# POSTECH-CVLab/InstaOrder

Measured on AMD Instinct MI355X. Metric: instance-pairs/sec (fwd+bwd), higher is better.
Workload: dtype f32; 1 GPU; InstaOrderNet_o, pair-batch 256 per GPU at 256x256x5, fp32, fwd+bwd+SGD (BASELINE.json configs[1]); inputs=resident in HBM, pairs_per_gpu=256, input_size=256, parallelism=dp1, hip_graph=True, setup_steps=0, inputs_distinct=True

## Files before the change

include/instaorder_hip.h:

```cpp
#ifndef INSTAORDER_HIP_H
#define INSTAORDER_HIP_H

#include <stddef.h>
#include <stdint.h>

#ifdef __cplusplus
extern "C" {
#endif

#define IO_OK 0
#define IO_ERR_SHAPE (-1)
#define IO_ERR_WORKSPACE (-2)
#define IO_ERR_LAUNCH (-3)
#define IO_ERR_STATE (-4)
#define IO_ERR_NODEVICE (-5)

#if !defined(__HIP__) && !defined(HIP_INCLUDE_HIP_HIP_RUNTIME_API_H)
typedef void* hipStream_t;
#endif

int io_abi_version(void);
const char* io_last_error_string(void);
int io_device_count(void);
int io_set_winograd(int on);
// ... 40 lines not shown
int io_maxpool_fwd(const float* x, int N, int H, int W, int C, float* out, uint32_t* idx, hipStream_t stream);
int io_maxpool_bwd(const float* dy, const uint32_t* idx, int N, int H, int W, int C, float* dx,
                   hipStream_t stream);
int io_avgpool_fc_fwd(const float* x, int N, int HW, int C, const float* w0, const float* b0, int K0,
                      const float* w1, const float* b1, int K1, float* pooled, float* logits, hipStream_t stream);
int io_avgpool_fc_bwd(const float* dlogits, const float* pooled, int N, int HW, int C, const float* w0, int K0,
                      const float* w1, int K1, const float* relu_mask, float* dx, float* dw0, float* db0, float* dw1,
                      float* db1, hipStream_t stream);

int io_pack_planes_nhwc8(const float* const* planes, const long* sample_strides, int nplanes, int N, int H, int W,
                         float* out, hipStream_t stream);

int io_order_loss(const float* logits, int N, int B, int Kocc, int Kdep, const float* occ_target,
                  const long* depth_target, const long* is_overlap, float overlap_weight, float distinct_weight,
                  float inv_world, float* losses, float* dlogits, hipStream_t stream);

int io_sgd_momentum(float* params, const float* grads, float* momentum_buf, size_t n, float lr, float momentum,
                    float weight_decay, hipStream_t stream);

int io_adam_step(float* params, const float* grads, float* exp_avg, float* exp_avg_sq, size_t n, double lr, double beta1,
                 double beta2, float eps, float weight_decay, double bias_correction1, double bias_correction2,
                 hipStream_t stream);

typedef struct io_clip_state {
    float norm;
    float coef;
    int nonfinite;
    int reserved0;
    uint64_t steps;
    uint64_t clipped;
    uint64_t skipped;
    uint64_t reserved[3];
} io_clip_state;
int io_grad_norm_chunk_floats(void);
size_t io_grad_norm_workspace_bytes(size_t n, int nseg);
int io_grad_norm(const float* grads, size_t n, const size_t* seg_offsets, int nseg, float max_norm, void* workspace,
                 size_t workspace_bytes, double* seg_sumsq, io_clip_state* state, hipStream_t stream);
int io_sgd_momentum_clipped(float* params, const float* grads, float* momentum_buf, size_t n, float lr, float momentum,
                            float weight_decay, const io_clip_state* clip, hipStream_t stream);
int io_adam_step_clipped(float* params, const float* grads, float* exp_avg, float* exp_avg_sq, size_t n, double lr,
                         double beta1, double beta2, float eps, float weight_decay, double bias_correction1,
                         double bias_correction2, const io_clip_state* clip, hipStream_t stream);

typedef struct io_net io_net;

typedef struct io_tensor_info {
    char name[64];
    int kind;
    int ndim;
    long shape[4];
    long offset;
    long numel_storage;
    int cin_storage;
    int bn_index;
    long running_offset;
} io_tensor_info;

io_net* io_net_create(int in_channels, int n_heads, const int* head_dims);
void io_net_destroy(io_net* net);
long io_net_param_floats(const io_net* net);
long io_net_running_floats(const io_net* net);
int io_net_num_tensors(const io_net* net);
int io_net_tensor_info(const io_net* net, int i, io_tensor_info* out);
int io_net_num_logits(const io_net* net);
size_t io_net_workspace_bytes(const io_net* net, int N, int S, int training);
long io_net_activation_offset(const io_net* net, int N, int S, int which);
int io_net_forward(io_net* net, const float* params, float* running, const void* x8, int N, int S, int G,
                   int training, void* workspace, size_t workspace_bytes, float* logits, hipStream_t stream);
size_t io_net_workspace_bytes_hw(const io_net* net, int N, int H, int W);
int io_net_forward_eval_hw(io_net* net, const float* params, float* running, const void* x8, int N, int H, int W,
                           void* workspace, size_t workspace_bytes, float* logits, hipStream_t stream);

int io_net_backward_num_stages(const io_net* net);
int io_net_backward_stages(io_net* net, const float* params, float* grads, const void* x8, const float* dlogits, int N,
                           int S, int G, void* workspace, size_t workspace_bytes, int stage_lo, int stage_hi,
                           hipStream_t stream);
int io_net_backward(io_net* net, const float* params, float* grads, const void* x8, const float* dlogits, int N,
                    int S, int G, void* workspace, size_t workspace_bytes, hipStream_t stream);

#define IO_DTYPE_F32 0
#define IO_DTYPE_BF16 1
int io_net_set_dtype(io_net* net, int dtype);
int io_net_get_dtype(const io_net* net);
int io_pack_planes_nhwc8_dt(const float* const* planes, const long* sample_strides, int nplanes, int N, int H, int W,
                            void* out, int dtype, hipStream_t stream);
int io_conv2d_fwd_dt(const void* x, const void* w, void* y, int N, int H, int W, int Cin, int Cout, int R, int S,
                     int stride, int pad, int dtype_in, int dtype_out, hipStream_t stream);
int io_conv2d_dgrad_dt(const void* dy, const void* wt, void* dx, const void* add, const void* relu_mask, int N, int H,
                       int W, int Cin, int Cout, int R, int S, int stride, int pad, int dtype, hipStream_t stream);
int io_conv2d_wgrad_dt(const void* x, const void* dy, float* dw, int N, int H, int W, int Cin, int Cout, int R, int S,
                       int stride, int pad, void* workspace, size_t workspace_bytes, int dtype_in, int dtype_dy,
                       hipStream_t stream);
int io_filter_prepare(const float* w, int Cout, int taps, int Cin, void* dst, int transpose, int dtype,
                      hipStream_t stream);
int io_bn_stats_finalize_dt(const void* y, int M, int C, int G, const float* gamma, const float* beta,
                            float* running_mean, float* running_var, float momentum, float eps, float* mean,
                            float* rstd, float* scale, float* shift, float* partial, size_t partial_floats, int dtype,
                            hipStream_t stream);
int io_bn_apply_bits_dt(const void* y, int M, int C, int G, int per_group_tables, const float* mean, const float* scale,
                        const float* shift, const void* identity, const float* mean2, const float* scale2,
                        const float* shift2, void* out, uint32_t* bits, int dtype, hipStream_t stream);
int io_bn_apply_dt(const void* y, int M, int C, int G, int per_group_tables, const float* mean, const float* scale,
                   const float* shift, const void* identity, const float* mean2, const float* scale2,
                   const float* shift2, int relu, void* out, int dtype, hipStream_t stream);
int io_bn_bwd_dt(const void* dout, const void* act, const float* mask_scale, const float* mask_shift, const void* y,
                 int M, int C, int G, const float* gamma, const float* mean, const float* rstd, float* dgamma,
                 float* dbeta, void* dy, void* dz_out, float* partial, size_t partial_floats, float* coef, int dtype,
                 hipStream_t stream);

int io_gconv_pack(const float* w, int C, int cg, int taps, void* wc, void* wtc, int dtype, hipStream_t stream);
int io_gconv_unpack_grad(const float* dwc, int C, int cg, int taps, float* dw, hipStream_t stream);
int io_gconv2d_fwd(const void* x, const void* wc, void* y, int N, int H, int W, int C, int R, int S, int stride, int pad,
                   int dtype, hipStream_t stream);
int io_gconv2d_dgrad(const void* dy, const void* wtc, void* dx, int N, int H, int W, int C, int R, int S, int stride,
                     int pad, int dtype, hipStream_t stream);
size_t io_gconv2d_wgrad_workspace_bytes(int N, int H, int W, int C, int R, int S, int stride, int pad);
int io_gconv2d_wgrad(const void* x, const void* dy, float* dwc, int N, int H, int W, int C, int R, int S, int stride,
                     int pad, void* workspace, size_t workspace_bytes, int dtype, hipStream_t stream);
int io_upsample2x_bilinear_fwd(const void* x, int N, int H, int W, int C, int align_corners, void* out, int dtype,
                               hipStream_t stream);
int io_upsample2x_bilinear_bwd(const void* dy, int N, int H, int W, int C, int align_corners, void* dx, int dtype,
                               hipStream_t stream);
int io_bias_act(const void* x, const float* bias, int M, int C, int relu, void* out, int dtype, hipStream_t stream);
int io_relu_bwd(const void* dy, const void* act, size_t n, void* dx, int dtype, hipStream_t stream);
int io_add(const void* a, const void* b, size_t n, void* out, int dtype, hipStream_t stream);
size_t io_colsum_partial_floats(int M, int C);
int io_colsum(const void* x, int M, int C, float* out, float* partial, size_t partial_floats, int dtype,
              hipStream_t stream);
int io_head1_fwd(const void* x, int M, int pitch, int C, const float* w, const float* b, int relu, float* out, int dtype,
                 hipStream_t stream);
int io_head1_bwd(const float* dy, const float* out, const void* x, int M, int pitch, int C, const float* w, int relu,
                 void* dx, float* dw, float* db, float* partial, size_t partial_floats, int dtype, hipStream_t stream);
size_t io_smooth_loss_workspace_floats(int B, int H, int W);
int io_smooth_loss_fwd(const float* disp, const float* img, int B, int H, int W, float out_scale, float* loss, float* g,
                       float* workspace, size_t workspace_floats, hipStream_t stream);
int io_smooth_loss_bwd(const float* g, const float* workspace, const float* grad_out, float scale, int B, int H, int W,
                       int accumulate, float* ddisp, hipStream_t stream);
size_t io_disp_order_workspace_floats(int B, int H, int W);
int io_disp_order_count(const float* disp1, const float* disp2, const float* modal1, const float* modal2,
                        const long* depth_order1, const long* is_overlap, int B, int H, int W, int le_order,
                        float out_scale, float* out, float* workspace, size_t workspace_floats, hipStream_t stream);
size_t io_depth_errors_median_workspace_bytes(int B, int H, int W);
int io_depth_errors_median(const float* pred, const uint16_t* gt, int B, int H, int W, float gt_div, float min_depth,
                           float max_depth, double* out, float* medians, void* workspace, size_t workspace_bytes,
                           hipStream_t stream);
int io_disp_sample_points(const float* disp, int B, int H, int W, const int* points, float* values, int* decisions,
                          hipStream_t stream);
#define IO_MASK_NONZERO 0
#define IO_MASK_EQ1 1
#define IO_MASK_MAX_N 65535
int io_mask_pack(const uint8_t* masks, int n, int H, int W, int predicate, int dilate, uint32_t* bits, int64_t* stats,
                 hipStream_t stream);
int io_mask_pair_counts(const uint32_t* p_bits, int n_p, const uint32_t* q_bits, int n_q, int H, int W, int32_t* counts,
                        hipStream_t stream);
#define IO_DEPTH_SELECT_MEAN 0
#define IO_DEPTH_SELECT_MEDIAN 1
size_t io_instance_depth_select_workspace_bytes(int n, int H, int W);
int io_instance_depth_select(const float* disp, int H, int W, const uint8_t* masks, int n, int method, float* value, float* lo,
                             float* hi, int32_t* k, void* workspace, size_t workspace_bytes, hipStream_t stream);
int io_conv2d_fwd_bnstats_dt(const void* x, const void* w, void* y, int N, int H, int W, int Cin, int Cout, int R, int S,
                             int stride, int pad, int G, const float* gamma, const float* beta, float* running_mean,
                             float* running_var, float momentum, float eps, float* mean, float* rstd, float* scale,
                             float* shift, float* workspace, size_t workspace_floats, int dtype, int gw,
                             hipStream_t stream);
int io_conv2d_dgrad_bnbwd_dt(const void* dy, const void* wt, void* dz, int N, int H, int W, int Cin, int Cout, int R, int S,
                             int pad, const void* y, int G, const float* gamma, const float* mean, const float* rstd,
                             const float* scale, const float* shift, float* dgamma, float* dbeta, void* dyb,
                             float* workspace, size_t workspace_floats, int dtype, int gw, hipStream_t stream);
size_t io_stem_packed_floats(int real_channels);
size_t io_stem_wgrad_exact_workspace_bytes(int N, int H, int W, int real_channels);
int io_stem_fwd_bnstats_exact(const float* x8, const float* w, float* y, int N, int H, int W, int real_channels, int G,
                              const float* gamma, const float* beta, float* running_mean, float* running_var,
                              float momentum, float eps, float* mean, float* rstd, float* scale, float* shift,
                              float* workspace, size_t workspace_floats, float* packed, hipStream_t stream);
int io_stem_wgrad_exact(const float* x8, const float* dy, float* dw, int N, int H, int W, int real_channels,
                        void* workspace, size_t workspace_bytes, float* packed, hipStream_t stream);
int io_stem_wgrad_exact_bn(const float* x8, const float* da, const float* y, float* dw, int N, int H, int W,
                           int real_channels, int G, const float* gamma, const float* mean, const float* rstd,
                           const float* scale, const float* shift, float* dgamma, float* dbeta, float* coef,
                           float* bn_partial, size_t bn_partial_floats, void* workspace, size_t workspace_bytes,
                           float* packed, hipStream_t stream);

size_t io_bn_tile_partial_floats(int M, int C, int G);
int io_bn_bwd_coefs_dt(const void* dz, const void* y, int M, int C, int G, const float* gamma, const float* mean,
                       const float* rstd, float* dgamma, float* dbeta, float* coef, float* partial,
                       size_t partial_floats, int dtype, hipStream_t stream);
int io_bn_bwd_coefs_from_tile_partials(float* p1, float* p2, int M, int C, int G, const float* gamma, const float* mean,
                                       const float* rstd, float* dgamma, float* dbeta, float* coef, hipStream_t stream);
typedef struct io_dgrad_fused {
    const void* xb_y;
    const float* xb_coef;
    void* xb_dy_out;
    const void* add;
    const void* relu_mask;
    const void* ep_y;
    const float *ep_mean, *ep_rstd, *ep_scale, *ep_shift;
    void* ep_act_out;
    float *ep_p1, *ep_p2;
    float* wino_scratch;
    size_t wino_scratch_floats;
    const uint32_t* relu_maskbits;
} io_dgrad_fused;
int io_conv2d_dgrad_fused_dt(const void* dy, const void* wt, void* dx, int N, int H, int W, int Cin, int Cout, int R,
                             int S, int pad, int G, const io_dgrad_fused* f, int dtype, hipStream_t stream);
size_t io_conv2d_wino_scratch_floats(int Cin, int Cout);
int io_conv2d_fwd_wino(const float* x, const float* w, float* y, int N, int H, int W, int Cin, int Cout, int G,
                       const float* in_mean, const float* in_scale, const float* in_shift, const float* gamma,
                       const float* beta, float* running_mean, float* running_var, float momentum, float eps, float* mean,
                       float* rstd, float* scale, float* shift, float* workspace, size_t workspace_floats,
                       float* wino_scratch, size_t wino_floats, hipStream_t stream);
int io_conv2d_fwd_xf_dt(const void* x, const void* w, void* y, int N, int H, int W, int Cin, int Cout, int R, int S,
                        int stride, int pad, int G, const float* in_mean, const float* in_scale, const float* in_shift,
                        const float* gamma, const float* beta, float* running_mean, float* running_var, float momentum, float eps,
                        float* mean, float* rstd, float* scale, float* shift, float* workspace, size_t workspace_floats,
                        int dtype, hipStream_t stream);
int io_conv2d_fwd_resid(const float* y3, const float* identity, const float* w, float* y, float* out, int N, int H, int W,
                        int Cin, int Cout, int G, const float* in_mean, const float* in_scale, const float* in_shift,
                        const float* gamma, const float* beta, float* running_mean, float* running_var, float momentum,
                        float eps, float* mean, float* rstd, float* scale, float* shift, float* workspace,
                        size_t workspace_floats, hipStream_t stream);
int io_conv2d_fwd_resid_dt(const void* y3, const void* second, const void* w, void* y, void* out, uint32_t* out_bits, int N,
                           int H, int W, int Cin, int Cout, int G, int two, const float* ta, const float* tb, const float* tc,
                           float* tile_mean, float* tile_m2, int dtype, hipStream_t stream);
int io_set_bf16_p256_xop(int on);
int io_get_bf16_p256_xop(void);
typedef struct io_weight_desc {
    long src, dst_op, dst_t, dst_g;
    int Co, Ci, T, Cop, Cip;
} io_weight_desc;
int io_weights_prepare(const void* table, int n, const float* params, void* ops, int dtype, hipStream_t stream);
int io_weights_unpack_grads(const void* table, int n, const float* gk, float* grads, hipStream_t stream);
size_t io_stem_wgrad_bf16_workspace_bytes(void);
int io_stem_wgrad_bn_bf16(const void* x8, const void* da, const void* y, float* dw, int N, int H, int W, int G,
                          const float* gamma, const float* mean, const float* rstd, const float* scale, const float* shift,
                          float* dgamma, float* dbeta, float* coef, float* bn_partial, size_t bn_partial_floats,
                          void* workspace, size_t workspace_bytes, hipStream_t stream);
int io_debug_last_wgrad_route(void);
int io_maxpool_fwd_xf_dt(const void* x, int N, int H, int W, int C, void* out, uint32_t* idx, int G,
                         const float* in_mean, const float* in_scale, const float* in_shift, int dtype,
                         hipStream_t stream);
int io_conv2d_fwd_bias_dt(const void* x, const void* w, void* y, int N, int H, int W, int Cin, int Cout, int R, int S,
                          int stride, int pad, const float* bias, const void* add, int relu, int dtype, int gw,
                          hipStream_t stream);
int io_maxpool_fwd_dt(const void* x, int N, int H, int W, int C, void* out, uint32_t* idx, int dtype, hipStream_t stream);
int io_maxpool_bwd_dt(const void* dy, const uint32_t* idx, int N, int H, int W, int C, void* dx, int dtype,
                      hipStream_t stream);
int io_avgpool_fc_fwd_dt(const void* x, int N, int HW, int C, const float* w0, const float* b0, int K0, const float* w1,
                         const float* b1, int K1, float* pooled, float* logits, int dtype, hipStream_t stream);
int io_avgpool_fc_bwd_dt(const float* dlogits, const float* pooled, int N, int HW, int C, const float* w0, int K0,
                         const float* w1, int K1, const void* relu_mask, void* dx, float* dw0, float* db0, float* dw1,
                         float* db1, int dtype, hipStream_t stream);

typedef struct io_pair_desc {
    int64_t image_off;
    int64_t mask1_off, mask2_off;
    int32_t H, W;
    int32_t x, y, w, h;
    int32_t flip;
    int32_t interp;
} io_pair_desc;
int io_pair_planes_u8(const uint8_t* arena, size_t arena_bytes, const io_pair_desc* desc_dev,
                      const io_pair_desc* desc_host, int P, int S, const double* mean3, const double* std3, float* rgb,
                      float* modal1, float* modal2, hipStream_t stream);
int io_pair_planes_u8_hw(const uint8_t* arena, size_t arena_bytes, const io_pair_desc* desc_dev,
// ... 33 lines not shown
```

instaorder_amd/_lib.py:

```python
import ctypes as C
import os

_HERE = os.path.dirname(os.path.abspath(__file__))
LIB_PATH = os.environ.get("IO_LIB_PATH") or os.path.join(_HERE, "libinstaorder_hip.so")
_lib = None

c_float_p = C.c_void_p


def csrc_digest():
    import glob
    import hashlib
    h = hashlib.sha256()
    files = sorted(glob.glob(os.path.join(_HERE, "csrc", "*.hip")) + glob.glob(os.path.join(_HERE, "csrc", "*.h")))
    files.append(os.path.join(os.path.dirname(_HERE), "include", "instaorder_hip.h"))
    for f in files:
        h.update(os.path.basename(f).encode())
        h.update(open(f, "rb").read())
    return h.hexdigest()[:16]


class TensorInfo(C.Structure):
    _fields_ = [("name", C.c_char * 64), ("kind", C.c_int), ("ndim", C.c_int), ("shape", C.c_long * 4),
                ("offset", C.c_long), ("numel_storage", C.c_long), ("cin_storage", C.c_int),
# ... 11 lines not shown
                ("value", C.c_int32), ("out_off", C.c_int64)]


class DgradFused(C.Structure):
    _fields_ = [(n, C.c_void_p) for n in ("xb_y", "xb_coef", "xb_dy_out", "add", "relu_mask", "ep_y", "ep_mean", "ep_rstd",
                                          "ep_scale", "ep_shift", "ep_act_out", "ep_p1", "ep_p2", "wino_scratch")] + \
               [("wino_scratch_floats", C.c_size_t), ("relu_maskbits", C.c_void_p)]


class ProfEntry(C.Structure):
    _fields_ = [("name", C.c_char * 48), ("launches", C.c_long), ("total_ms", C.c_double),
                ("flops", C.c_double), ("bytes", C.c_double), ("flops_executed", C.c_double)]


class ClipState(C.Structure):
    _fields_ = [("norm", C.c_float), ("coef", C.c_float), ("nonfinite", C.c_int), ("reserved0", C.c_int),
                ("steps", C.c_uint64), ("clipped", C.c_uint64), ("skipped", C.c_uint64), ("reserved", C.c_uint64 * 3)]


_P, _I, _L, _F, _Z = C.c_void_p, C.c_int, C.c_long, C.c_float, C.c_size_t
_D = C.c_double

SIGNATURES = {
    "io_abi_version": (_I, []),
    "io_last_error_string": (C.c_char_p, []),
    "io_device_count": (_I, []),
    "io_set_winograd": (_I, [_I]),
    "io_get_winograd": (_I, []),
    "io_set_bf16_p256": (_I, [_I]),
    "io_get_bf16_p256": (_I, []),
    "io_set_bf16_p256_xop": (_I, [_I]),
    "io_get_bf16_p256_xop": (_I, []),
    "io_conv2d_fwd_resid_dt": (_I, [_P, _P, _P, _P, _P, _P, _I, _I, _I, _I, _I, _I, _I, _P, _P, _P, _P, _P, _I, _P]),
    "io_debug_last_nt_route": (_I, []),
    "io_conv2d_fwd": (_I, [_P, _P, _P, _I, _I, _I, _I, _I, _I, _I, _I, _I, _P]),
    "io_conv2d_bnstats_workspace_floats": (_Z, [_I, _I, _I, _I, _I, _I, _I, _I, _I]),
    "io_conv2d_fwd_bnstats": (_I, [_P, _P, _P, _I, _I, _I, _I, _I, _I, _I, _I, _I, _I, _P, _P, _P, _P, _F, _F, _P, _P,
                                   _P, _P, _P, _Z, _P]),
    "io_conv2d_dgrad": (_I, [_P, _P, _P, _P, _P, _I, _I, _I, _I, _I, _I, _I, _I, _I, _P]),
    "io_conv2d_dgrad_bnbwd": (_I, [_P, _P, _P, _I, _I, _I, _I, _I, _I, _I, _I, _P, _I, _P, _P, _P, _P, _P, _P, _P, _P,
                                   _P, _Z, _P]),
    "io_conv2d_wgrad_workspace_bytes": (_Z, [_I, _I, _I, _I, _I, _I, _I, _I, _I]),
    "io_conv2d_wgrad": (_I, [_P, _P, _P, _I, _I, _I, _I, _I, _I, _I, _I, _I, _P, _Z, _P]),
    "io_filter_transpose": (_I, [_P, _I, _I, _I, _P, _P]),
    "io_bn_partial_floats": (_Z, [_I, _I, _I]),
    "io_bn_stats_finalize": (_I, [_P, _I, _I, _I, _P, _P, _P, _P, _F, _F, _P, _P, _P, _P, _P, _Z, _P]),
    "io_bn_eval_prepare": (_I, [_I, _P, _P, _P, _P, _F, _P, _P, _P, _P]),
    "io_bn_apply": (_I, [_P, _I, _I, _I, _I, _P, _P, _P, _P, _P, _P, _P, _I, _P, _P]),
    "io_bn_bwd": (_I, [_P, _P, _P, _P, _P, _I, _I, _I, _P, _P, _P, _P, _P, _P, _P, _P, _Z, _P, _P]),
    "io_maxpool_fwd": (_I, [_P, _I, _I, _I, _I, _P, _P, _P]),
    "io_maxpool_bwd": (_I, [_P, _P, _I, _I, _I, _I, _P, _P]),
    "io_avgpool_fc_fwd": (_I, [_P, _I, _I, _I, _P, _P, _I, _P, _P, _I, _P, _P, _P]),
    "io_avgpool_fc_bwd": (_I, [_P, _P, _I, _I, _I, _P, _I, _P, _I, _P, _P, _P, _P, _P, _P, _P]),
    "io_pack_planes_nhwc8": (_I, [C.POINTER(C.c_void_p), C.POINTER(C.c_long), _I, _I, _I, _I, _P, _P]),
    "io_pair_planes_u8": (_I, [_P, _Z, _P, _P, _I, _I, _P, _P, _P, _P, _P, _P]),
    "io_pair_planes_u8_hw": (_I, [_P, _Z, _P, _P, _I, _I, _I, _P, _P, _P, _P, _P, _P]),
    "io_rle_decode_u8": (_I, [_P, _Z, _P, _P, _I, _P, _Z, _P]),
    "io_rle_lds_runs": (_I, []),
    "io_order_loss": (_I, [_P, _I, _I, _I, _I, _P, _P, _P, _F, _F, _F, _P, _P, _P]),
    "io_sgd_momentum": (_I, [_P, _P, _P, _Z, _F, _F, _F, _P]),
    "io_adam_step": (_I, [_P, _P, _P, _P, _Z, _D, _D, _D, _F, _F, _D, _D, _P]),
    "io_grad_norm": (_I, [_P, _Z, C.POINTER(C.c_size_t), _I, _F, _P, _Z, _P, _P, _P]),
    "io_grad_norm_workspace_bytes": (_Z, [_Z, _I]),
    "io_grad_norm_chunk_floats": (_I, []),
    "io_sgd_momentum_clipped": (_I, [_P, _P, _P, _Z, _F, _F, _F, _P, _P]),
    "io_adam_step_clipped": (_I, [_P, _P, _P, _P, _Z, _D, _D, _D, _F, _F, _D, _D, _P, _P]),
    "io_net_create": (_P, [_I, _I, C.POINTER(C.c_int)]),
    "io_net_destroy": (None, [_P]),
    "io_net_param_floats": (_L, [_P]),
    "io_net_running_floats": (_L, [_P]),
    "io_net_num_tensors": (_I, [_P]),
    "io_net_tensor_info": (_I, [_P, _I, C.POINTER(TensorInfo)]),
    "io_net_num_logits": (_I, [_P]),
    "io_net_workspace_bytes": (_Z, [_P, _I, _I, _I]),
    "io_net_workspace_bytes_hw": (_Z, [_P, _I, _I, _I]),
    "io_net_forward_eval_hw": (_I, [_P, _P, _P, _P, _I, _I, _I, _P, _Z, _P, _P]),
    "io_net_activation_offset": (_L, [_P, _I, _I, _I]),
    "io_net_forward": (_I, [_P, _P, _P, _P, _I, _I, _I, _I, _P, _Z, _P, _P]),
    "io_net_backward": (_I, [_P, _P, _P, _P, _P, _I, _I, _I, _P, _Z, _P]),
    "io_net_backward_num_stages": (_I, [_P]),
    "io_net_backward_stages": (_I, [_P, _P, _P, _P, _P, _I, _I, _I, _P, _Z, _I, _I, _P]),
    "io_net_set_dtype": (_I, [_P, _I]),
    "io_net_get_dtype": (_I, [_P]),
    "io_pack_planes_nhwc8_dt": (_I, [_P, _P, _I, _I, _I, _I, _P, _I, _P]),
    "io_conv2d_fwd_dt": (_I, [_P, _P, _P, _I, _I, _I, _I, _I, _I, _I, _I, _I, _I, _I, _P]),
    "io_conv2d_dgrad_dt": (_I, [_P, _P, _P, _P, _P, _I, _I, _I, _I, _I, _I, _I, _I, _I, _I, _P]),
    "io_conv2d_wgrad_dt": (_I, [_P, _P, _P, _I, _I, _I, _I, _I, _I, _I, _I, _I, _P, _Z, _I, _I, _P]),
    "io_filter_prepare": (_I, [_P, _I, _I, _I, _P, _I, _I, _P]),
    "io_bn_stats_finalize_dt": (_I, [_P, _I, _I, _I, _P, _P, _P, _P, _F, _F, _P, _P, _P, _P, _P, _Z, _I, _P]),
    "io_bn_apply_dt": (_I, [_P, _I, _I, _I, _I, _P, _P, _P, _P, _P, _P, _P, _I, _P, _I, _P]),
    "io_bn_apply_bits_dt": (_I, [_P, _I, _I, _I, _I, _P, _P, _P, _P, _P, _P, _P, _P, _P, _I, _P]),
    "io_bn_bwd_dt": (_I, [_P, _P, _P, _P, _P, _I, _I, _I, _P, _P, _P, _P, _P, _P, _P, _P, _Z, _P, _I, _P]),
    "io_gconv_pack": (_I, [_P, _I, _I, _I, _P, _P, _I, _P]),
    "io_gconv_unpack_grad": (_I, [_P, _I, _I, _I, _P, _P]),
    "io_gconv2d_fwd": (_I, [_P, _P, _P, _I, _I, _I, _I, _I, _I, _I, _I, _I, _P]),
    "io_gconv2d_dgrad": (_I, [_P, _P, _P, _I, _I, _I, _I, _I, _I, _I, _I, _I, _P]),
    "io_gconv2d_wgrad_workspace_bytes": (_Z, [_I, _I, _I, _I, _I, _I, _I, _I]),
    "io_gconv2d_wgrad": (_I, [_P, _P, _P, _I, _I, _I, _I, _I, _I, _I, _I, _P, _Z, _I, _P]),
    "io_upsample2x_bilinear_fwd": (_I, [_P, _I, _I, _I, _I, _I, _P, _I, _P]),
    "io_upsample2x_bilinear_bwd": (_I, [_P, _I, _I, _I, _I, _I, _P, _I, _P]),
    "io_bias_act": (_I, [_P, _P, _I, _I, _I, _P, _I, _P]),
    "io_relu_bwd": (_I, [_P, _P, _Z, _P, _I, _P]),
    "io_add": (_I, [_P, _P, _Z, _P, _I, _P]),
    "io_colsum_partial_floats": (_Z, [_I, _I]),
    "io_colsum": (_I, [_P, _I, _I, _P, _P, _Z, _I, _P]),
    "io_head1_fwd": (_I, [_P, _I, _I, _I, _P, _P, _I, _P, _I, _P]),
    "io_head1_bwd": (_I, [_P, _P, _P, _I, _I, _I, _P, _I, _P, _P, _P, _P, _Z, _I, _P]),
    "io_conv2d_fwd_bnstats_dt": (_I, [_P, _P, _P, _I, _I, _I, _I, _I, _I, _I, _I, _I, _I, _P, _P, _P, _P, _F, _F, _P,
                                      _P, _P, _P, _P, _Z, _I, _I, _P]),
    "io_conv2d_fwd_bias_dt": (_I, [_P, _P, _P, _I, _I, _I, _I, _I, _I, _I, _I, _I, _P, _P, _I, _I, _I, _P]),
    "io_stem_packed_floats": (_Z, [_I]),
    "io_stem_wgrad_exact_workspace_bytes": (_Z, [_I, _I, _I, _I]),
    "io_stem_fwd_bnstats_exact": (_I, [_P, _P, _P, _I, _I, _I, _I, _I, _P, _P, _P, _P, _F, _F, _P, _P, _P, _P, _P, _Z, _P,
                                       _P]),
    "io_stem_wgrad_exact": (_I, [_P, _P, _P, _I, _I, _I, _I, _P, _Z, _P, _P]),
    "io_stem_wgrad_exact_bn": (_I, [_P, _P, _P, _P, _I, _I, _I, _I, _I, _P, _P, _P, _P, _P, _P, _P, _P, _P, _Z, _P, _Z, _P,
                                    _P]),
    "io_stem_wgrad_bn_bf16": (_I, [_P, _P, _P, _P, _I, _I, _I, _I, _P, _P, _P, _P, _P, _P, _P, _P, _P, _Z, _P, _Z, _P]),
    "io_stem_wgrad_bf16_workspace_bytes": (_Z, []),
    "io_debug_last_wgrad_route": (_I, []),
    "io_conv2d_fwd_resid": (_I, [_P, _P, _P, _P, _P, _I, _I, _I, _I, _I, _I, _P, _P, _P, _P, _P, _P, _P, _F, _F, _P, _P, _P,
                                 _P, _P, _Z, _P]),
    "io_smooth_loss_workspace_floats": (_Z, [_I, _I, _I]),
    "io_smooth_loss_fwd": (_I, [_P, _P, _I, _I, _I, _F, _P, _P, _P, _Z, _P]),
    "io_smooth_loss_bwd": (_I, [_P, _P, _P, _F, _I, _I, _I, _I, _P, _P]),
    "io_disp_order_workspace_floats": (_Z, [_I, _I, _I]),
    "io_disp_order_count": (_I, [_P, _P, _P, _P, _P, _P, _I, _I, _I, _I, _F, _P, _P, _Z, _P]),
    "io_bn_tile_partial_floats": (_Z, [_I, _I, _I]),
    "io_bn_bwd_coefs_dt": (_I, [_P, _P, _I, _I, _I, _P, _P, _P, _P, _P, _P, _P, _Z, _I, _P]),
    "io_bn_bwd_coefs_from_tile_partials": (_I, [_P, _P, _I, _I, _I, _P, _P, _P, _P, _P, _P, _P]),
    "io_conv2d_dgrad_fused_dt": (_I, [_P, _P, _P, _I, _I, _I, _I, _I, _I, _I, _I, _I, C.POINTER(DgradFused), _I, _P]),
    "io_conv2d_dgrad_bnbwd_dt": (_I, [_P, _P, _P, _I, _I, _I, _I, _I, _I, _I, _I, _P, _I, _P, _P, _P, _P, _P, _P, _P, _P, _P,
                                      _Z, _I, _I, _P]),
    "io_prof_launches": (_I, [_P, _I]),
    "io_weights_prepare": (_I, [_P, _I, _P, _P, _I, _P]),
    "io_weights_unpack_grads": (_I, [_P, _I, _P, _P, _P]),
    "io_maxpool_fwd_xf_dt": (_I, [_P, _I, _I, _I, _I, _P, _P, _I, _P, _P, _P, _I, _P]),
    "io_conv2d_fwd_xf_dt": (_I, [_P, _P, _P, _I, _I, _I, _I, _I, _I, _I, _I, _I, _I, _P, _P, _P, _P, _P, _P, _P, _F, _F, _P,
                                 _P, _P, _P, _P, _Z, _I, _P]),
    "io_conv2d_wino_scratch_floats": (_Z, [_I, _I]),
    "io_conv2d_fwd_wino": (_I, [_P, _P, _P, _I, _I, _I, _I, _I, _I, _P, _P, _P, _P, _P, _P, _P, _F, _F, _P, _P, _P, _P, _P, _Z,
                                _P, _Z, _P]),
    "io_maxpool_fwd_dt": (_I, [_P, _I, _I, _I, _I, _P, _P, _I, _P]),
    "io_maxpool_bwd_dt": (_I, [_P, _P, _I, _I, _I, _I, _P, _I, _P]),
    "io_avgpool_fc_fwd_dt": (_I, [_P, _I, _I, _I, _P, _P, _I, _P, _P, _I, _P, _P, _I, _P]),
    "io_avgpool_fc_bwd_dt": (_I, [_P, _P, _I, _I, _I, _P, _I, _P, _I, _P, _P, _P, _P, _P, _P, _I, _P]),
    "io_depth_errors_median_workspace_bytes": (_Z, [_I, _I, _I]),
    "io_depth_errors_median": (_I, [_P, _P, _I, _I, _I, _F, _F, _F, _P, _P, _P, _Z, _P]),
    "io_disp_sample_points": (_I, [_P, _I, _I, _I, _P, _P, _P, _P]),
    "io_mask_pack": (_I, [_P, _I, _I, _I, _I, _I, _P, _P, _P]),
    "io_mask_pair_counts": (_I, [_P, _I, _P, _I, _I, _I, _P, _P]),
    "io_instance_depth_select_workspace_bytes": (_Z, [_I, _I, _I]),
    "io_instance_depth_select": (_I, [_P, _I, _I, _P, _I, _I, _P, _P, _P, _P, _P, _Z, _P]),
    "io_prof_begin": (_I, []),
    "io_prof_begin_ex": (_I, [_I]),
    "io_prof_end": (_I, [C.POINTER(ProfEntry), _I]),
}


def lib():
    global _lib
    if _lib is None:
        if not os.path.isfile(LIB_PATH):
            raise RuntimeError(
                "instaorder_amd: %s is missing -- the HIP extension has not been built "
                "(run `make -C instaorder_amd/csrc`). There is no CPU fallback." % LIB_PATH)
        _lib = C.CDLL(LIB_PATH)
        for name, (res, args) in SIGNATURES.items():
            fn = getattr(_lib, name)
            fn.restype = res
            fn.argtypes = args
    return _lib


def last_error():
    return lib().io_last_error_string().decode()


def check(rc, what):
    if rc != 0:
        raise RuntimeError("instaorder_hip %s failed (%d): %s" % (what, rc, last_error()))


_gpu_ok = None


def require_gpu():
    global _gpu_ok
    if _gpu_ok is None:
        _gpu_ok = lib().io_device_count() > 0
    if not _gpu_ok:
        raise RuntimeError("instaorder_amd: no gfx950 (MI355X) device visible; the HIP path cannot run "
                           "and there is no CPU fallback")
```

instaorder_amd/csrc/capi.hip:

```cpp
#include <stdarg.h>
#include <stdio.h>
#include <stdlib.h>
#include <string.h>

#include "io_common.h"

static thread_local char g_err[512] = "";

void io_set_error(const char* fmt, ...) {
    va_list ap;
    va_start(ap, fmt);
    vsnprintf(g_err, sizeof(g_err), fmt, ap);
    va_end(ap);
}

int io_check_launch(const char* what) {
    hipError_t e = hipGetLastError();
    if (e != hipSuccess) {
        io_set_error("%s: %s", what, hipGetErrorString(e));
        return IO_ERR_LAUNCH;
    }
    return IO_OK;
}

// ... 364 lines not shown
                                    float* db0, float* dw1, float* db1, int dtype, hipStream_t st) {
    IO_REQUIRE(dtype == IO_F32 || dtype == IO_BF16, IO_ERR_SHAPE, "avgpool_fc: unknown dtype %d", dtype);
    return io_avgpool_fc_bwd_t(dlogits, pooled, N, HW, C, w0, K0, w1, K1, relu_mask, dx, dw0, db0, dw1, db1, st, dtype);
}


extern "C" int io_conv2d_fwd_bnstats_dt(const void* x, const void* w, void* y, int N, int H, int W, int Cin, int Cout,
                                        int R, int S, int stride, int pad, int G, const float* gamma, const float* beta,
                                        float* running_mean, float* running_var, float momentum, float eps, float* mean,
                                        float* rstd, float* scale, float* shift, float* workspace,
                                        size_t workspace_floats, int dtype, int gw, hipStream_t st) {
    IO_REQUIRE(dtype == IO_F32 || dtype == IO_BF16, IO_ERR_SHAPE, "conv2d_fwd_bnstats: unknown dtype %d", dtype);
    IoConvGeom g = io_geom_fwd(N, H, W, Cin, Cout, R, S, stride, pad);
    g.gw = gw;
    const int M = N * g.Ho * g.Wo;
    IO_REQUIRE(G >= 1 && M % G == 0 && (M / G) % kIoStatTileRows == 0, IO_ERR_SHAPE,
               "conv2d_fwd_bnstats: rows per BN group (%d) must be a multiple of %d", G ? M / G : 0, kIoStatTileRows);
    const size_t need = io_conv2d_bnstats_workspace_floats(N, H, W, Cout, R, S, stride, pad, G);
    IO_REQUIRE(workspace_floats >= need, IO_ERR_WORKSPACE, "conv2d_fwd_bnstats: workspace %zu < %zu floats",
               workspace_floats, need);
    float* tmean = workspace;
    float* tm2 = workspace + need / 2;
    int rc = io_launch_conv_nt(g, x, w, y, nullptr, nullptr, Cin == 8, st, tmean, tm2, nullptr, dtype, dtype);
    if (rc) return rc;
    return io_bn_finalize_tiles(tmean, tm2, M, Cout, G, gamma, beta, running_mean, running_var, momentum, eps, mean,
                                rstd, scale, shift, st);
}


extern "C" int io_conv2d_dgrad_bnbwd_dt(const void* dy, const void* wt, void* dz, int N, int H, int W, int Cin, int Cout,
                                        int R, int S, int pad, const void* y, int G, const float* gamma, const float* mean,
                                        const float* rstd, const float* scale, const float* shift, float* dgamma,
                                        float* dbeta, void* dyb, float* workspace, size_t workspace_floats, int dtype,
                                        int gw, hipStream_t st) {
    IO_REQUIRE(dtype == IO_F32 || dtype == IO_BF16, IO_ERR_SHAPE, "conv2d_dgrad_bnbwd: unknown dtype %d", dtype);
    IO_REQUIRE(Cin % 64 == 0, IO_ERR_SHAPE, "conv2d_dgrad_bnbwd: Cin=%d must be a multiple of 64", Cin);
    const int M = N * H * W;
    IO_REQUIRE(G >= 1 && M % G == 0 && (M / G) % kIoStatTileRows == 0, IO_ERR_SHAPE,
               "conv2d_dgrad_bnbwd: rows per BN group (%d) must be a multiple of %d", G ? M / G : 0, kIoStatTileRows);
    const size_t tiles = (size_t)M / kIoStatTileRows;
    const size_t per = (tiles + tiles / 64 + G + 2) * (size_t)Cin;
    IO_REQUIRE(workspace_floats >= 2 * per + 2 * (size_t)G * Cin, IO_ERR_WORKSPACE,
               "conv2d_dgrad_bnbwd: workspace %zu < %zu floats", workspace_floats, 2 * per + 2 * (size_t)G * Cin);
    IoBwStats bw{};
    bw.y = y; bw.mean = mean; bw.rstd = rstd; bw.mscale = scale; bw.mshift = shift;
    bw.p1 = workspace; bw.p2 = workspace + per; bw.Mg = M / G;
    int rc = io_run_dgrad(dy, wt, dz, nullptr, nullptr, N, H, W, Cin, Cout, R, S, 1, pad, st, &bw, dtype, gw);
    if (rc) return rc;
    return io_bn_bwd_from_tiles(bw.p1, bw.p2, dz, y, M, Cin, G, gamma, mean, rstd, dgamma, dbeta, dyb,
                                workspace + 2 * per, st, dtype);
}

extern "C" size_t io_stem_packed_floats(int real_channels) { return (size_t)64 * io_stem_kp(49, real_channels); }
static IoConvGeom stem_geom_exact(int N, int H, int W, int cr) {
    IoConvGeom g = io_geom_fwd(N, H, W, 8, 64, 7, 7, 2, 3);
    g.cr = cr;
    return g;
}
extern "C" size_t io_stem_wgrad_exact_workspace_bytes(int N, int H, int W, int real_channels) {
    return io_conv_wgrad_partial_bytes(stem_geom_exact(N, H, W, real_channels), 1);
}
extern "C" int io_stem_fwd_bnstats_exact(const float* x8, const float* w, float* y, int N, int H, int W, int real_channels,
                                         int G, const float* gamma, const float* beta, float* running_mean,
                                         float* running_var, float momentum, float eps, float* mean, float* rstd,
                                         float* scale, float* shift, float* workspace, size_t workspace_floats,
                                         float* packed, hipStream_t st) {
    IO_REQUIRE(real_channels >= 1 && real_channels <= 8, IO_ERR_SHAPE, "stem_exact: real_channels=%d (1..8)", real_channels);
    IoConvGeom g = stem_geom_exact(N, H, W, real_channels);
    const int M = N * g.Ho * g.Wo;
    IO_REQUIRE(G >= 1 && M % G == 0 && (M / G) % kIoStatTileRows == 0, IO_ERR_SHAPE,
               "stem_exact: rows per BN group (%d) must be a multiple of %d", G ? M / G : 0, kIoStatTileRows);
    const size_t need = io_conv2d_bnstats_workspace_floats(N, H, W, 64, 7, 7, 2, 3, G);
    IO_REQUIRE(workspace_floats >= need && packed, IO_ERR_WORKSPACE, "stem_exact: workspace %zu < %zu floats",
               workspace_floats, need);
    int rc = io_stem_pack_filter(w, packed, 64, 49, real_channels, st);
    if (rc) return rc;
    float* tmean = workspace;
    float* tm2 = workspace + need / 2;
    rc = io_launch_conv_nt(g, x8, packed, y, nullptr, nullptr, 1, st, tmean, tm2);
    if (rc) return rc;
    return io_bn_finalize_tiles(tmean, tm2, M, 64, G, gamma, beta, running_mean, running_var, momentum, eps, mean, rstd,
                                scale, shift, st);
}
extern "C" int io_stem_wgrad_exact(const float* x8, const float* dy, float* dw, int N, int H, int W, int real_channels,
                                   void* ws, size_t ws_bytes, float* packed, hipStream_t st) {
    IO_REQUIRE(real_channels >= 1 && real_channels <= 8 && packed, IO_ERR_SHAPE, "stem_wgrad_exact: real_channels=%d (1..8)",
               real_channels);
    IoConvGeom g = stem_geom_exact(N, H, W, real_channels);
    int rc = io_launch_conv_wgrad(g, x8, dy, packed, (float*)ws, ws_bytes, 1, st);
    if (rc) return rc;
    return io_stem_unpack_grad(packed, dw, 64, 49, real_channels, st);
}

extern "C" int io_stem_wgrad_exact_bn(const float* x8, const float* da, const float* y, float* dw, int N, int H, int W,
                                      int real_channels, int G, const float* gamma, const float* mean, const float* rstd,
                                      const float* scale, const float* shift, float* dgamma, float* dbeta, float* coef,
                                      float* bn_partial, size_t bn_partial_floats, void* ws, size_t ws_bytes, float* packed,
                                      hipStream_t st) {
    IO_REQUIRE(real_channels >= 1 && real_channels <= 8 && packed && coef, IO_ERR_SHAPE,
               "stem_wgrad_exact_bn: real_channels=%d (1..8)", real_channels);
    IoConvGeom g = stem_geom_exact(N, H, W, real_channels);
    IO_REQUIRE(io_stem_rows_ok(g) && G >= 1 && N % G == 0, IO_ERR_SHAPE,
               "stem_wgrad_exact_bn: needs 5 real channels, 256 | H, W and G | N (else: io_bn_bwd + io_stem_wgrad_exact)");
    const int M = N * g.Ho * g.Wo;
    int rc = io_bn_bwd_coefs_t(da, y, M, 64, G, gamma, mean, rstd, dgamma, dbeta, coef, bn_partial, bn_partial_floats, st, IO_F32,
                               scale, shift);
    if (rc) return rc;
    IoStemXb xb{};
    xb.y = y;
    xb.a = coef;
    xb.b = coef + (size_t)G * 64;
    xb.c = coef + (size_t)2 * G * 64;
    xb.mean = mean;
    xb.scale = scale;
    xb.shift = shift;
    xb.G = G;
    rc = io_launch_stem_wgrad_rows(g, x8, da, packed, (float*)ws, ws_bytes, st, &xb);
    if (rc) return rc;
    return io_stem_unpack_grad(packed, dw, 64, 49, real_channels, st);
}

extern "C" size_t io_stem_wgrad_bf16_workspace_bytes(void) { return io_stem_wgrad_halo_partial_bytes(); }
extern "C" int io_stem_wgrad_bn_bf16(const void* x8, const void* da, const void* y, float* dw, int N, int H, int W, int G,
                                     const float* gamma, const float* mean, const float* rstd, const float* scale,
                                     const float* shift, float* dgamma, float* dbeta, float* coef, float* bn_partial,
                                     size_t bn_partial_floats, void* ws, size_t ws_bytes, hipStream_t st) {
    IO_REQUIRE(x8 && da && y && dw && coef && ws, IO_ERR_SHAPE, "stem_wgrad_bn_bf16: null argument");
    IoConvGeom g = io_geom_fwd(N, H, W, 8, 64, 7, 7, 2, 3);
    IO_REQUIRE(io_stem_wgrad_halo_ok(g, ws_bytes, G), IO_ERR_SHAPE,
               "stem_wgrad_bn_bf16: needs 256 x 256 inputs (128-wide output rows), G | N, io_stem_wgrad_bf16_workspace_bytes() of "
               "workspace and enough rows for the persistent blocks (else: io_bn_bwd_dt + io_conv2d_wgrad_dt)");
    const int M = N * g.Ho * g.Wo;
    int rc = io_bn_bwd_coefs_t(da, y, M, 64, G, gamma, mean, rstd, dgamma, dbeta, coef, bn_partial, bn_partial_floats, st, IO_BF16,
                               scale, shift);
    if (rc) return rc;
    IoStemXb xb{};
    xb.y = (const float*)y;
    xb.a = coef;
    xb.b = coef + (size_t)G * 64;
    xb.c = coef + (size_t)2 * G * 64;
    xb.mean = mean;
    xb.scale = scale;
    xb.shift = shift;
    xb.G = G;
    return io_launch_stem_wgrad_halo(g, x8, da, dw, (float*)ws, ws_bytes, st, &xb);
}

extern "C" size_t io_bn_tile_partial_floats(int M, int C, int G) {
    if (M <= 0 || C <= 0 || G <= 0) return 0;
    const size_t tiles = (size_t)(M + kIoStatTileRows - 1) / kIoStatTileRows;
    return (tiles + tiles / 64 + (size_t)G + 2) * (size_t)C;
}

extern "C" int io_bn_bwd_coefs_dt(const void* dz, const void* y, int M, int C, int G, const float* gamma, const float* mean,
                                  const float* rstd, float* dgamma, float* dbeta, float* coef, float* partial,
                                  size_t partial_floats, int dtype, hipStream_t st) {
    IO_REQUIRE(dtype == IO_F32 || dtype == IO_BF16, IO_ERR_SHAPE, "bn_bwd_coefs: unknown dtype %d", dtype);
    return io_bn_bwd_coefs_t(dz, y, M, C, G, gamma, mean, rstd, dgamma, dbeta, coef, partial, partial_floats, st, dtype);
}

extern "C" int io_bn_bwd_coefs_from_tile_partials(float* p1, float* p2, int M, int C, int G, const float* gamma,
                                                  const float* mean, const float* rstd, float* dgamma, float* dbeta,
                                                  float* coef, hipStream_t st) {
    return io_bn_bwd_coefs_from_tiles(p1, p2, M, C, G, gamma, mean, rstd, dgamma, dbeta, coef, st);
}

extern "C" int io_conv2d_dgrad_fused_dt(const void* dy, const void* wt, void* dx, int N, int H, int W, int Cin, int Cout,
                                        int R, int S, int pad, int G, const io_dgrad_fused* f, int dtype, hipStream_t st) {
    IO_REQUIRE(dtype == IO_F32 || dtype == IO_BF16, IO_ERR_SHAPE, "conv2d_dgrad_fused: unknown dtype %d", dtype);
    IO_REQUIRE(f != nullptr, IO_ERR_SHAPE, "conv2d_dgrad_fused: the option struct is required");
    IO_REQUIRE(Cin % 64 == 0, IO_ERR_SHAPE, "conv2d_dgrad_fused: Cin=%d must be a multiple of 64", Cin);
    const int M = N * H * W;
    const bool grouped = f->xb_coef || f->ep_y;
    IO_REQUIRE(!grouped || (G >= 1 && M % G == 0 && (M / G) % kIoStatTileRows == 0), IO_ERR_SHAPE,
               "conv2d_dgrad_fused: rows per BN group (%d) must be a multiple of %d", G ? M / G : 0, kIoStatTileRows);
    IO_REQUIRE(!f->xb_coef || f->xb_y, IO_ERR_SHAPE, "conv2d_dgrad_fused: xb_coef needs xb_y");
    IO_REQUIRE(!f->ep_y || (f->ep_mean && f->ep_rstd && f->ep_p1 && f->ep_p2 && (f->ep_scale == nullptr) == (f->ep_shift == nullptr)),
               IO_ERR_SHAPE, "conv2d_dgrad_fused: ep_y needs ep_mean / ep_rstd / ep_p1 / ep_p2 (and scale / shift as a pair)");
    IO_REQUIRE(!f->ep_act_out || (f->ep_y && f->ep_scale), IO_ERR_SHAPE,
               "conv2d_dgrad_fused: ep_act_out needs ep_y with ep_scale / ep_shift");
    IoBwStats bw{};
    if (f->ep_y) {
        bw.y = f->ep_y; bw.mean = f->ep_mean; bw.rstd = f->ep_rstd; bw.mscale = f->ep_scale; bw.mshift = f->ep_shift;
        bw.p1 = f->ep_p1; bw.p2 = f->ep_p2; bw.Mg = M / G; bw.a_out = f->ep_act_out;
    }
    if (f->xb_coef) {
        const size_t gs = (size_t)G * Cout;
        bw.xb_y = f->xb_y; bw.xb_a = f->xb_coef; bw.xb_b = f->xb_coef + gs; bw.xb_c = f->xb_coef + 2 * gs;
        bw.xb_out = f->xb_dy_out; bw.xb_Mg = M / G;
    }
    if (f->wino_scratch) {
        IO_REQUIRE(f->wino_scratch_floats >= io_conv2d_wino_scratch_floats(Cin, Cout), IO_ERR_WORKSPACE,
                   "conv2d_dgrad_fused: wino_scratch %zu < %zu floats", f->wino_scratch_floats,
                   io_conv2d_wino_scratch_floats(Cin, Cout));
        bw.wino_u = f->wino_scratch;
    }
    if (f->relu_maskbits) {
        IO_REQUIRE(f->relu_mask && Cin % 32 == 0, IO_ERR_SHAPE,
                   "conv2d_dgrad_fused: relu_maskbits goes WITH relu_mask (the same mask, one bit per element), 32 | Cin");
        bw.maskbits = f->relu_maskbits;
    }
    return io_run_dgrad(dy, wt, dx, f->add, f->relu_mask, N, H, W, Cin, Cout, R, S, 1, pad, st,
// ... 120 lines not shown
```

instaorder_amd/csrc/io_common.h:

```cpp
#pragma once
#include <hip/hip_runtime.h>
#include <stdint.h>
#include <stddef.h>

#include "../../include/instaorder_hip.h"

void io_set_error(const char* fmt, ...);
int io_check_launch(const char* what);

#define IO_REQUIRE(cond, code, ...)        \
    do {                                   \
        if (!(cond)) {                     \
            io_set_error(__VA_ARGS__);     \
            return (code);                 \
        }                                  \
    } while (0)

static inline int io_cdiv(long a, long b) { return (int)((a + b - 1) / b); }

#include <atomic>
static inline int io_device_cu_count() {
    static std::atomic<int> cache[64];
    int dev = 0;
    if (hipGetDevice(&dev) != hipSuccess || dev < 0 || dev >= 64) return 256;
// ... 89 lines not shown
    const void* y;
    const float *mean, *rstd, *mscale, *mshift;
    float *p1, *p2;
    int Mg;
    void* a_out;
    const float* bias;
    int relu;
    const float *in_mean, *in_scale, *in_shift;
    int in_Mg;
    const void* xb_y;
    const float *xb_a, *xb_b, *xb_c;
    void* xb_out;
    int xb_Mg;
    int xb_res;
    uint32_t* xb_bits;
    float* wino_u;
    const uint32_t* maskbits;
};

bool io_wino_on();

int io_launch_conv_nt(const IoConvGeom& g, const void* in, const void* wgt, void* out, const void* add,
                      const void* mask, int stem, hipStream_t st, float* st_mean = nullptr,
                      float* st_m2 = nullptr, const IoBwStats* bw = nullptr, int dt_in = IO_F32,
                      int dt_out = IO_F32);
bool io_conv_p256_takes_xop(long M, int Ci, int Co, int Mg);
int io_launch_conv_p256(const IoConvGeom& g, const void* in, const void* wgt, void* out, const void* add, const void* mask,
                        hipStream_t st, float* st_mean, float* st_m2, const IoBwStats* bw, size_t in_bytes,
                        unsigned w_bytes, size_t out_bytes);
int io_bf16_persist_mode();
int io_launch_conv_halo3(const IoConvGeom& g, const void* in, const void* wgt, void* out, const void* add, const void* mask,
                         hipStream_t st, float* st_mean, float* st_m2, const IoBwStats* bw, size_t in_bytes,
                         unsigned w_bytes, size_t out_bytes);
int io_launch_conv_stem_halo(const IoConvGeom& g, const void* in, const void* wgt, void* out, hipStream_t st, float* st_mean,
                             float* st_m2, const IoBwStats* bw, size_t in_bytes, unsigned w_bytes, size_t out_bytes);
int io_bn_bwd_from_tiles(float* p1, float* p2, const void* dz, const void* y, int M, int C, int G,
                         const float* gamma, const float* mean, const float* rstd, float* dgamma, float* dbeta,
                         void* dy, float* coef, hipStream_t st, int dt = IO_F32);
int io_bn_bwd_coefs_from_tiles(float* p1, float* p2, int M, int C, int G, const float* gamma, const float* mean,
                               const float* rstd, float* dgamma, float* dbeta, float* coef, hipStream_t st);
int io_bn_bwd_coefs_t(const void* dz, const void* y, int M, int C, int G, const float* gamma, const float* mean,
                      const float* rstd, float* dgamma, float* dbeta, float* coef, float* partial,
                      size_t partial_floats, hipStream_t st, int dt, const float* mask_scale = nullptr,
                      const float* mask_shift = nullptr);
int io_bn_stats_finalize_t(const void* y, int M, int C, int G, const float* gamma, const float* beta,
                           float* running_mean, float* running_var, float momentum, float eps, float* mean,
                           float* rstd, float* scale, float* shift, float* partial, size_t partial_floats,
                           hipStream_t st, int dt);
int io_bn_apply_t(const void* y, int M, int C, int G, int per_group_tables, const float* mean, const float* scale,
                  const float* shift, const void* identity, const float* mean2, const float* scale2,
                  const float* shift2, int relu, void* out, hipStream_t st, int dt, uint32_t* bits = nullptr);
int io_bn_bwd_t(const void* dout, const void* act, const float* mask_scale, const float* mask_shift, const void* y,
                int M, int C, int G, const float* gamma, const float* mean, const float* rstd, float* dgamma,
                float* dbeta, void* dy, void* dz_out, float* partial, size_t partial_floats, float* coef,
                hipStream_t st, int dt);
int io_maxpool_fwd_t(const void* x, int N, int H, int W, int C, void* out, uint32_t* idx, hipStream_t st, int dt,
                     const float* xs = nullptr, const float* xh = nullptr, int G = 1, const float* xm = nullptr);
int io_maxpool_bwd_t(const void* dy, const uint32_t* idx, int N, int H, int W, int C, void* dx, hipStream_t st, int dt);
int io_avgpool_fc_fwd_t(const void* x, int N, int HW, int C, const float* w0, const float* b0, int K0,
                        const float* w1, const float* b1, int K1, float* pooled, float* logits, hipStream_t st,
                        int dt);
int io_avgpool_fc_bwd_t(const float* dlogits, const float* pooled, int N, int HW, int C, const float* w0, int K0,
                        const float* w1, int K1, const void* relu_mask, void* dx, float* dw0, float* db0, float* dw1,
                        float* db1, hipStream_t st, int dt);
int io_pack_planes_t(const float* const* planes, const long* sample_strides, int nplanes, int N, int H, int W,
                     void* out, hipStream_t st, int dt);
int io_filter_prepare_t(const float* w, int O, int T, int C, void* dst, int transpose, hipStream_t st, int dt);
int io_stem_pack_filter(const float* w, float* wp, int O, int T, int cr, hipStream_t st);
int io_stem_unpack_grad(const float* dwp, float* dw, int O, int T, int cr, hipStream_t st);
int io_bn_resid2_tables(const float* mean3, const float* scale3, const float* shift3, const float* meand,
                        const float* scaled, const float* shiftd, int G, int C, float* coef, hipStream_t st);
constexpr int kIoStatTileRows = 128;
int io_bn_finalize_tiles(float* tile_mean, float* tile_m2, int M, int C, int G, const float* gamma,
                         const float* beta, float* running_mean, float* running_var, float momentum, float eps,
                         float* mean, float* rstd, float* scale, float* shift, hipStream_t st);
int io_launch_conv_wgrad(const IoConvGeom& g, const void* in, const void* dy, float* dw, float* partial,
                         size_t partial_bytes, int stem, hipStream_t st, int dt_in = IO_F32, int dt_dy = IO_F32);
size_t io_conv_wgrad_partial_bytes(const IoConvGeom& g, int stem);

IoConvGeom io_geom_fwd(int N, int H, int W, int Cin, int Cout, int R, int S, int stride, int pad);
bool io_stem_rows_ok(const IoConvGeom& g);
int io_launch_stem_rows(const IoConvGeom& g, const float* x8, const float* wp, float* out, float* st_mean, float* st_m2,
                        const float* bias, int relu, hipStream_t st);
int io_stem_wgrad_rows_max_blocks();
struct IoStemXb {
    const float *y, *a, *b, *c, *mean, *scale, *shift;
    int G, tiles_per_group;
};
int io_launch_stem_wgrad_rows(const IoConvGeom& g, const float* x8, const float* dy, float* dwp, float* partial,
                              size_t partial_bytes, hipStream_t st, const IoStemXb* xb = nullptr);
size_t io_stem_wgrad_halo_partial_bytes();
bool io_stem_wgrad_halo_ok(const IoConvGeom& g, size_t partial_bytes, int G);
int io_launch_stem_wgrad_halo(const IoConvGeom& g, const void* x8, const void* dz, float* dw, float* partial, size_t partial_bytes,
                              hipStream_t st, const IoStemXb* xb);
size_t io_wgrad_halo3_partial_bytes();
bool io_wgrad_halo3_shape(const IoConvGeom& g);
int io_launch_conv_wgrad_halo3(const IoConvGeom& g, const void* x, const void* dy, float* dw, float* partial, size_t partial_bytes,
                               hipStream_t st);
int io_splitk_reduce(const float* partial, float* dst, size_t n4, int splits, hipStream_t st);
struct IoFilterTable {
    static constexpr int kMax = 64;
    int n;
    int start[kMax + 1];
    int O[kMax], T[kMax], C[kMax];
    unsigned off[kMax];
};
int io_filter_table_add(IoFilterTable& tab, long off, int O, int T, int C);
int io_filter_transpose_all(const IoFilterTable& tab, const float* params, void* wt_all, hipStream_t st, int dt);
IoConvGeom io_geom_dgrad(int N, int H, int W, int Cin, int Cout, int R, int S, int stride, int pad, int ph, int pw);
int io_run_dgrad(const void* dy, const void* wt, void* dx, const void* add, const void* mask, int N, int H,
                 int W, int Cin, int Cout, int R, int S, int stride, int pad, hipStream_t st,
                 const IoBwStats* bw = nullptr, int dt = IO_F32, int gw = 0);

enum IoProfClass {
    IO_PROF_CONV_NT128 = 0, IO_PROF_CONV_NT64, IO_PROF_CONV_STEM, IO_PROF_WGRAD, IO_PROF_WGRAD_STEM,
    IO_PROF_BN_STATS, IO_PROF_BN_APPLY, IO_PROF_BN_BWD, IO_PROF_POOL_HEAD, IO_PROF_TRANSPOSE, IO_PROF_PACK,
    IO_PROF_LOSS, IO_PROF_SGD, IO_PROF_CONV_WINO, IO_PROF_WGRAD_WINO, IO_PROF_ADAM, IO_PROF_GRAD_NORM,
    IO_PROF_RLE, IO_PROF_NCLASS
};
struct IoProfScope {
    int idx;
    hipStream_t st;
    IoProfScope(int cls, double flops, double bytes, hipStream_t stream, double flops_exec = -1.0);
    ~IoProfScope();
};
```

instaorder_amd/csrc/misc.hip:

```cpp
#include "io_common.h"

#ifndef IO_POOL_ROWS
#define IO_POOL_ROWS 1
#endif

namespace {

constexpr int kThreads = 256;

template <typename T> __device__ __forceinline__ f32x4 ld4(const T* p) { return io_ldv(p); }
template <typename T> __device__ __forceinline__ void st4(T* p, f32x4 v) { io_stv(p, v); }
__device__ __forceinline__ float ld1(const float* p) { return *p; }
__device__ __forceinline__ float ld1(const bf16_t* p) { return io_bf2f(*p); }
__device__ __forceinline__ void st1(float* p, float v) { *p = v; }
__device__ __forceinline__ void st1(bf16_t* p, float v) { *p = io_f2bf(v); }

int ew_blocks(size_t n) {
    size_t b = (n + kThreads - 1) / kThreads;
    return (int)(b > 8192 ? 8192 : (b ? b : 1));
}

struct PackArgs {
    const float* plane[5];
    long stride[5];
// ... 871 lines not shown
extern "C" size_t io_grad_norm_workspace_bytes(size_t n, int nseg) {
    return ((n + kNormChunk - 1) / kNormChunk + (size_t)(nseg > 0 ? nseg : 0)) * sizeof(double);
}

extern "C" int io_grad_norm(const float* grads, size_t n, const size_t* seg_offsets, int nseg, float max_norm,
                            void* workspace, size_t workspace_bytes, double* seg_sumsq, io_clip_state* state,
                            hipStream_t st) {
    static_assert(sizeof(io_clip_state) == 64, "io_clip_state is a 64-byte record");
    NormTable tab;
    const int rc = norm_table(tab, n, seg_offsets, nseg);
    if (rc != IO_OK) return rc;
    IO_REQUIRE(max_norm > 0.f, IO_ERR_SHAPE, "grad_norm: max_norm=%g must be > 0 (+inf: measure only)", (double)max_norm);
    IO_REQUIRE(seg_sumsq && state && (grads || n == 0), IO_ERR_SHAPE, "grad_norm: null pointer");
    const size_t blocks = (size_t)tab.start[nseg];
    IO_REQUIRE(blocks == 0 || (workspace && workspace_bytes >= blocks * sizeof(double)), IO_ERR_SHAPE,
               "grad_norm: workspace of %zu bytes, %zu needed", workspace_bytes, blocks * sizeof(double));
    IO_REQUIRE(((uintptr_t)grads & 15) == 0 && ((uintptr_t)workspace & 7) == 0, IO_ERR_SHAPE,
               "grad_norm: grads must be 16-byte aligned, the workspace 8-byte aligned");
    IoProfScope prof(IO_PROF_GRAD_NORM, 3.0 * n, 4.0 * n, st);
    if (blocks)
        hipLaunchKernelGGL(grad_norm_partial_kernel, dim3((unsigned)blocks), dim3(kThreads), 0, st, tab, grads,
                           (double*)workspace);
    hipLaunchKernelGGL(grad_norm_fold_kernel, dim3(1), dim3(kThreads), 0, st, tab, (const double*)workspace, seg_sumsq,
                       max_norm, state);
    return io_check_launch("grad_norm");
}

int io_filter_prepare_t(const float* w, int O, int T, int C, void* dst, int transpose, hipStream_t st, int dt) {
    IoProfScope prof(IO_PROF_TRANSPOSE, 0.0, (4.0 + io_dtype_bytes(dt)) * O * T * C, st);
    if (transpose) {
        dim3 grid(io_cdiv(C, 32), io_cdiv(O, 32), T);
        if (dt == IO_BF16)
            hipLaunchKernelGGL(filter_transpose_kernel<bf16_t>, grid, dim3(256), 0, st, w, O, T, C, (bf16_t*)dst);
        else
            hipLaunchKernelGGL(filter_transpose_kernel<float>, grid, dim3(256), 0, st, w, O, T, C, (float*)dst);
    } else {
        IO_REQUIRE(dt == IO_BF16 && ((size_t)O * T * C) % 4 == 0, IO_ERR_SHAPE, "filter_prepare: nothing to do");
        const size_t n4 = (size_t)O * T * C / 4;
        hipLaunchKernelGGL(cast_bf16_kernel, dim3(ew_blocks(n4)), dim3(kThreads), 0, st, w, (bf16_t*)dst, n4);
    }
    return io_check_launch("filter_prepare");
}

int io_filter_table_add(IoFilterTable& tab, long off, int O, int T, int C) {
    IO_REQUIRE(tab.n < IoFilterTable::kMax && off >= 0 && off < (1L << 32) && off % 8 == 0 && O > 0 && T > 0 && C > 0,
               IO_ERR_SHAPE, "filter table: entry %d (offset %ld, %d x %d x %d)", tab.n, off, O, T, C);
    const int l = tab.n++;
    tab.off[l] = (unsigned)off;
    tab.O[l] = O; tab.T[l] = T; tab.C[l] = C;
    tab.start[l + 1] = tab.start[l] + io_cdiv(C, 32) * io_cdiv(O, 32) * T;
    return IO_OK;
}

int io_filter_transpose_all(const IoFilterTable& tab, const float* params, void* wt_all, hipStream_t st, int dt) {
    if (tab.n == 0) return IO_OK;
    double elems = 0.0;
    for (int l = 0; l < tab.n; ++l) elems += (double)tab.O[l] * tab.T[l] * tab.C[l];
    IoProfScope prof(IO_PROF_TRANSPOSE, 0.0, (4.0 + io_dtype_bytes(dt)) * elems, st);
    const dim3 grid((unsigned)tab.start[tab.n]);
    if (dt == IO_BF16)
        hipLaunchKernelGGL(filter_transpose_all_kernel<bf16_t>, grid, dim3(256), 0, st, tab, params, (bf16_t*)wt_all);
    else
        hipLaunchKernelGGL(filter_transpose_all_kernel<float>, grid, dim3(256), 0, st, tab, params, (float*)wt_all);
    return io_check_launch("filter_transpose_all");
}

namespace {
__global__ __launch_bounds__(256) void stem_pack_filter_kernel(const float* __restrict__ w, float* __restrict__ wp,
                                                              int O, int T, int cr, int kp) {
    const int idx = blockIdx.x * 256 + threadIdx.x;
    if (idx >= O * kp) return;
    const int o = idx / kp, k = idx - o * kp;
    const int tp = k / cr, ch = k - tp * cr;
    wp[idx] = tp < T ? w[((size_t)o * T + tp) * 8 + ch] : 0.f;
}
__global__ __launch_bounds__(256) void stem_unpack_grad_kernel(const float* __restrict__ dwp, float* __restrict__ dw,
                                                              int O, int T, int cr, int kp) {
    const int idx = blockIdx.x * 256 + threadIdx.x;
    if (idx >= O * T * 8) return;
    const int ch = idx & 7, ot = idx >> 3;
    const int o = ot / T, tp = ot - o * T;
    dw[idx] = ch < cr ? dwp[(size_t)o * kp + tp * cr + ch] : 0.f;
}
}

int io_stem_pack_filter(const float* w, float* wp, int O, int T, int cr, hipStream_t st) {
    const int kp = io_stem_kp(T, cr);
    hipLaunchKernelGGL(stem_pack_filter_kernel, dim3(io_cdiv((long)O * kp, 256)), dim3(256), 0, st, w, wp, O, T, cr, kp);
    return io_check_launch("stem_pack_filter");
}

int io_stem_unpack_grad(const float* dwp, float* dw, int O, int T, int cr, hipStream_t st) {
    const int kp = io_stem_kp(T, cr);
    hipLaunchKernelGGL(stem_unpack_grad_kernel, dim3(io_cdiv((long)O * T * 8, 256)), dim3(256), 0, st, dwp, dw, O, T,
                       cr, kp);
    return io_check_launch("stem_unpack_grad");
}

extern "C" int io_filter_transpose(const float* w, int O, int T, int C, float* wt, hipStream_t st) {
    return io_filter_prepare_t(w, O, T, C, wt, 1, st, IO_F32);
}
```

instaorder_amd/csrc/net.hip:

```cpp
#include <stdio.h>
#include <string.h>

#include <vector>

#include "io_common.h"

namespace {

constexpr int kMaxGroups = 8;
constexpr float kBnEps = 1e-5f, kBnMomentum = 0.1f;

struct ConvL {
    int cin, cout, k, stride, pad, cin_store;
    long w_off;
};
struct BnL {
    int C;
    long g_off, b_off, run_off;
    int index;
};
struct Block {
    ConvL c1, c2, c3, cd;
    BnL b1, b2, b3, bd;
    bool down;
    int stride, inC, planes;
};

inline size_t align_up(size_t v, size_t a) { return (v + a - 1) / a * a; }

}

struct io_net {
    int dtype = IO_F32;
    int in_ch, n_heads, head_dims[2];
    ConvL stem;
    BnL bn1;
    std::vector<Block> blocks;
    long fcw_off[2], fcb_off[2];
    long param_floats, running_floats;
    int n_bn;
    long bn_channels;
    std::vector<io_tensor_info> tensors;
};

namespace {

void add_tensor(io_net* net, const char* name, int kind, int ndim, const long* shape, long numel_storage,
                int cin_storage, long* off_out, int bn_index = -1, long run_off = -1) {
    io_tensor_info t;
    memset(&t, 0, sizeof(t));
    snprintf(t.name, sizeof(t.name), "%s", name);
    t.kind = kind;
    t.ndim = ndim;
    for (int i = 0; i < ndim; ++i) t.shape[i] = shape[i];
    t.offset = net->param_floats;
    t.numel_storage = numel_storage;
    t.cin_storage = cin_storage;
    t.bn_index = bn_index;
    t.running_offset = run_off;
    *off_out = net->param_floats;
    net->param_floats = (long)align_up((size_t)(net->param_floats + numel_storage), 64);
    net->tensors.push_back(t);
}

ConvL add_conv(io_net* net, const char* name, int cout, int cin, int k, int stride, int pad) {
    ConvL c;
    c.cin = cin; c.cout = cout; c.k = k; c.stride = stride; c.pad = pad;
    c.cin_store = (cin % 32 == 0) ? cin : 8;
    char nm[64];
    snprintf(nm, sizeof(nm), "%s.weight", name);
    const long shape[4] = {cout, cin, k, k};
    add_tensor(net, nm, 0, 4, shape, (long)cout * k * k * c.cin_store, c.cin_store, &c.w_off);
    return c;
}

BnL add_bn(io_net* net, const char* name, int C) {
    BnL b;
    b.C = C;
    b.index = net->n_bn++;
    b.run_off = net->running_floats;
    net->running_floats += 2L * C;
    net->bn_channels += C;
    char nm[64];
    const long shape[1] = {C};
    snprintf(nm, sizeof(nm), "%s.weight", name);
    add_tensor(net, nm, 1, 1, shape, C, C, &b.g_off, b.index, b.run_off);
    snprintf(nm, sizeof(nm), "%s.bias", name);
    add_tensor(net, nm, 2, 1, shape, C, C, &b.b_off, b.index, b.run_off);
    return b;
}

constexpr size_t kNoBuf = ~(size_t)0;
struct BlockBufs {
    size_t y1, a1, y2, a2, y3, yd, out;
    size_t bits;
};
struct Plan {
    size_t y0, a0, p0, idx0, pooled;
    std::vector<BlockBufs> blk;
    size_t tables;
    size_t bn_partial, bn_partial_floats, coef;
    size_t tile_mean, tile_m2;
    size_t gbuf[5];
    size_t aside;
    size_t wt, wg_partial, wg_partial_bytes;
    size_t wop;
    size_t stem_wp, stem_dwp;
    size_t wt_all;
    size_t wfold, fbias;
    size_t wino_u;
    size_t total;
};

struct Arena {
    size_t top = 0;
    size_t take(size_t bytes) {
// ... 98 lines not shown
        p.wg_partial_bytes = 0;
    }
    p.total = a.top;
    return p;
}

struct FoldDesc {
    long w_off, g_off, b_off, run_off, bias_off;
    int rows, rowlen;
};
struct FoldTable {
    int n;
    FoldDesc d[56];
};
template <typename T>
__global__ __launch_bounds__(256) void fold_bn_kernel(FoldTable t, const float* __restrict__ params,
                                                     const float* __restrict__ running, float eps,
                                                     T* __restrict__ wout, float* __restrict__ bias) {
    const FoldDesc d = t.d[blockIdx.y];
    for (int row = blockIdx.x; row < d.rows; row += gridDim.x) {
        const float s = params[d.g_off + row] / sqrtf(running[d.run_off + d.rows + row] + eps);
        if (threadIdx.x == 0) bias[d.bias_off + row] = params[d.b_off + row] - running[d.run_off + row] * s;
        const float* src = params + d.w_off + (size_t)row * d.rowlen;
        T* dst = wout + d.w_off + (size_t)row * d.rowlen;
        for (int k = threadIdx.x; k < d.rowlen; k += 256) {
            if constexpr (sizeof(T) == 2) dst[k] = io_f2bf(src[k] * s);
            else dst[k] = src[k] * s;
        }
    }
}

#define IO_TRY(expr)            \
    do {                        \
        int rc_ = (expr);       \
        if (rc_) return rc_;    \
    } while (0)

struct Tables {
    float *mean, *rstd, *scale, *shift;
};

struct Ctx {
    const io_net* net;
    const float* params;
    float* running;
    float* grads;
    char* ws;
    Plan plan;
    int N, S, G;
    int SW;
    bool training;
    hipStream_t st;
    std::vector<long> chan_prefix;

    float* buf(size_t off) const { return reinterpret_cast<float*>(ws + off); }
    void* act(size_t off) const { return ws + off; }
    int dt() const { return net->dtype; }
    const void* wop(long w_off) const {
        return net->dtype == IO_BF16 ? (const void*)(reinterpret_cast<const bf16_t*>(ws + plan.wop) + w_off)
                                     : (const void*)(params + w_off);
    }
    const void* wfold(long w_off) const {
        return net->dtype == IO_BF16 ? (const void*)(reinterpret_cast<const bf16_t*>(ws + plan.wfold) + w_off)
                                     : (const void*)(reinterpret_cast<const float*>(ws + plan.wfold) + w_off);
    }
    float* fbias(const BnL& b) const { return buf(plan.fbias) + chan_prefix[b.index]; }
    Tables tables(const BnL& b) const {
        float* base = buf(plan.tables) + (size_t)4 * kMaxGroups * chan_prefix[b.index];
        const size_t gs = (size_t)kMaxGroups * b.C;
        return Tables{base, base + gs, base + 2 * gs, base + 3 * gs};
    }
};

bool stem_exact(const Ctx& c, const ConvL& L) { return L.cin_store == 8 && c.net->dtype == IO_F32; }

int conv_fwd(const Ctx& c, const ConvL& L, const void* x, void* y, int H, bool stats = false, const BnL* xf = nullptr,
             int Mout = 0, const BnL* xr = nullptr, const void* xr_id = nullptr, void* xr_out = nullptr,
             bool xr_two = false, uint32_t* xr_bits = nullptr) {
    IoConvGeom g = io_geom_fwd(c.N, H, H, L.cin_store, L.cout, L.k, L.k, L.stride, L.pad);
    const bool stem = L.cin_store == 8;
    const void* w = c.wop(L.w_off);
    if (stem_exact(c, L)) {
        g.cr = L.cin;
        IO_TRY(io_stem_pack_filter(c.params + L.w_off, c.buf(c.plan.stem_wp), L.cout, L.k * L.k, L.cin, c.st));
        w = c.buf(c.plan.stem_wp);
    }
    IoBwStats ep{};
    if (xf) {
        Tables t = c.tables(*xf);
        ep.in_mean = t.mean;
        ep.in_scale = t.scale;
        ep.in_shift = t.shift;
        ep.in_Mg = Mout / c.G;
    }
    const bool wino = c.plan.wino_u != kNoBuf && L.k == 3 && L.stride == 1 && c.dt() == IO_F32;
    if (wino) ep.wino_u = c.buf(c.plan.wino_u);
    if (xr) {
        Tables t = c.tables(*xr);
        ep.xb_y = xr_id;
        ep.xb_a = t.scale;
        ep.xb_b = t.mean;
        ep.xb_c = t.shift;
        ep.xb_out = xr_out;
        ep.xb_Mg = Mout / c.G;
        ep.xb_res = 1;
        ep.xb_bits = xr_bits;
        if (xr_two) {
            const size_t gs = (size_t)c.G * xr->C;
            ep.xb_a = c.buf(c.plan.coef);
            ep.xb_b = c.buf(c.plan.coef) + gs;
            ep.xb_c = c.buf(c.plan.coef) + 2 * gs;
            ep.xb_res = 2;
        }
    }
    return io_launch_conv_nt(g, x, w, y, nullptr, nullptr, stem, c.st,
                             stats ? c.buf(c.plan.tile_mean) : nullptr, stats ? c.buf(c.plan.tile_m2) : nullptr,
                             (xf || xr || wino) ? &ep : nullptr, c.dt(), c.dt());
}

int bn_prepare(const Ctx& c, const BnL& b, const void* y, int M, bool from_tiles = false) {
    Tables t = c.tables(b);
    if (c.training && from_tiles)
        return io_bn_finalize_tiles(c.buf(c.plan.tile_mean), c.buf(c.plan.tile_m2), M, b.C, c.G,
                                    c.params + b.g_off, c.params + b.b_off, c.running + b.run_off,
                                    c.running + b.run_off + b.C, kBnMomentum, kBnEps, t.mean, t.rstd, t.scale,
                                    t.shift, c.st);
    if (c.training)
        return io_bn_stats_finalize_t(y, M, b.C, c.G, c.params + b.g_off, c.params + b.b_off, c.running + b.run_off,
                                      c.running + b.run_off + b.C, kBnMomentum, kBnEps, t.mean, t.rstd, t.scale,
                                      t.shift, c.buf(c.plan.bn_partial), c.plan.bn_partial_floats, c.st, c.dt());
    return io_bn_eval_prepare(b.C, c.params + b.g_off, c.params + b.b_off, c.running + b.run_off,
                              c.running + b.run_off + b.C, kBnEps, t.mean, t.scale, t.shift, c.st);
}

int conv_bn(const Ctx& c, const ConvL& L, const BnL& b, const void* x, void* y, int Hin, int Mout,
            const BnL* xf = nullptr, const BnL* xr = nullptr, const void* xr_id = nullptr, void* xr_out = nullptr,
            bool xr_two = false, uint32_t* xr_bits = nullptr) {
    const bool fuse = c.training && (Mout / c.G) % kIoStatTileRows == 0;
    IO_TRY(conv_fwd(c, L, x, y, Hin, fuse, xf, Mout, xr, xr_id, xr_out, xr_two, xr_bits));
    return bn_prepare(c, b, y, Mout, fuse);
}

#ifndef IO_XB_BF16_MAXP
#define IO_XB_BF16_MAXP 64
#endif
#ifndef IO_XB_BF16_L1
#define IO_XB_BF16_L1 1
#endif
int out_rows(const Ctx& c, size_t i) {
    int H = c.S / 4;
    for (size_t k = 0; k <= i; ++k) H /= c.net->blocks[k].stride;
    return c.N * H * H;
}
int xr_route(const Ctx& c, size_t i) {
    if (!c.training || i + 1 >= c.net->blocks.size()) return 0;
    const Block& b = c.net->blocks[i];
    const int Mout = out_rows(c, i);
    if (Mout % c.G != 0 || (Mout / c.G) % kIoStatTileRows != 0) return 0;
    if (c.net->dtype == IO_F32) return 1;
    if (IO_XB_BF16_L1 && b.planes <= IO_XB_BF16_MAXP) return 1;
    return io_conv_p256_takes_xop(Mout, b.planes * 4, c.net->blocks[i + 1].planes, Mout / c.G) ? 2 : 0;
}

uint32_t* bits_of(const Ctx& c, size_t i) {
    const size_t off = c.plan.blk[i].bits;
    return (c.training && off != kNoBuf) ? reinterpret_cast<uint32_t*>(c.ws + off) : nullptr;
// ... 326 lines not shown
        if (stage_of[ii] < stage_lo || stage_of[ii] >= stage_hi) {
            have_tiles = ii > 0 && tiles_ok(c, Min);
            void* t = Gd; Gd = Ge; Ge = t;
            continue;
        }
        const void* xin = ii == 0 ? c.act(p.p0) : c.act(p.blk[ii - 1].out);
        const void* xmask = ii == 0 ? nullptr : xin;
        const bool x3p = c.net->dtype == IO_BF16 && b.planes > IO_XB_BF16_MAXP && tiles_ok(c, Mout) &&
                         io_conv_p256_takes_xop(Mout, b.planes * 4, b.planes, Mout / c.G);
        const bool x3 = xb_ok(c, Mout) || x3p ||
                        (IO_XB_BF16_L1 && c.net->dtype == IO_BF16 && b.planes <= IO_XB_BF16_MAXP && tiles_ok(c, Mout));
        const bool f3 = fuse_in(c, Mout), f2 = f3 && b.stride == 1;
        const bool x1d = b.stride == 1 && xb_ok(c, Min) && tiles_ok(c, Mout);
        const bool x1s = b.stride != 1 && xb_ok(c, Min) && bb.a1 != kNoBuf;
        const bool x1 = x1d || x1s;
        if (x3)
            IO_TRY(bn_back_coefs(c, b.b3, Gd, c.act(bb.y3), Mout, have_tiles));
        else if (have_tiles)
            IO_TRY(bn_back_tiles(c, b.b3, Gd, c.act(bb.y3), Mout, Ga));
        else
            IO_TRY(bn_back(c, b.b3, Gd, 0, nullptr, c.act(bb.y3), Mout, Ga, nullptr));
        have_tiles = false;
        void* As = f3 ? c.act(p.aside) : nullptr;
        if (!f3 && !x3) IO_TRY(conv_wgrad(c, b.c3, c.act(bb.a2), Ga, Ho));
        IO_TRY(dgrad_then_bn(c, b.c3, x3 ? Gd : Ga, Gb, Ho, b.b2, c.act(bb.y2), Mout, Gc, f3 ? As : nullptr,
                             x3 ? &b.b3 : nullptr, c.act(bb.y3), Mout, Ga));
        if (f3 || x3) IO_TRY(conv_wgrad(c, b.c3, f3 ? As : c.act(bb.a2), Ga, Ho));
        if (!f2) IO_TRY(conv_wgrad(c, b.c2, c.act(bb.a1), Gc, H));
        if (x1s)
            IO_TRY(conv_dgrad(c, b.c2, Gc, Ga, nullptr, c.act(bb.a1), H));
        else
            IO_TRY(dgrad_then_bn(c, b.c2, Gc, Ga, H, b.b1, c.act(bb.y1), Min, x1 ? nullptr : Gb, f2 ? As : nullptr));
        if (f2) IO_TRY(conv_wgrad(c, b.c2, As, Gc, H));
        if (!x1) IO_TRY(conv_wgrad(c, b.c1, xin, Gb, H));
        const void* partial = Gd;
        if (b.down && x3 && !x3p) {
            IO_TRY(bn_back_coefs(c, b.bd, Gd, c.act(bb.yd), Mout, false));
            IoBwStats bw{};
            xb_fill(c, bw, b.bd, c.act(bb.yd), Mout, Gc);
            IO_TRY(conv_dgrad(c, b.cd, Gd, Ge, nullptr, nullptr, H, &bw));
            IO_TRY(conv_wgrad(c, b.cd, xin, Gc, H));
            partial = Ge;
        } else if (b.down) {
            IO_TRY(bn_back(c, b.bd, Gd, 0, nullptr, c.act(bb.yd), Mout, Gc, nullptr));
            IO_TRY(conv_wgrad(c, b.cd, xin, Gc, H));
            IO_TRY(conv_dgrad(c, b.cd, Gc, Ge, nullptr, nullptr, H));
            partial = Ge;
        }
        if (x1) IO_TRY(bn_back_coefs(c, b.b1, Ga, c.act(bb.y1), Min, x1d));
        {
            IoBwStats bw{};
            const bool carry = ii > 0 && tiles_ok(c, Min);
            if (carry) bw = bw_for(c, net->blocks[ii - 1].b3, c.act(p.blk[ii - 1].y3), Min, false);
            if (x1) xb_fill(c, bw, b.b1, c.act(bb.y1), Min, Gb);
            const uint32_t* mbits = (ii > 0 && xmask && bits_written(c, ii - 1)) ? bits_of(c, ii - 1) : nullptr;
            if (mbits) bw.maskbits = mbits;
            IO_TRY(conv_dgrad(c, b.c1, x1 ? Ga : Gb, Ge, partial, xmask, H, (carry || x1 || mbits) ? &bw : nullptr));
            have_tiles = carry;
        }
        if (x1) IO_TRY(conv_wgrad(c, b.c1, xin, Gb, H));
        void* t = Gd; Gd = Ge; Ge = t;
    }
    if (stage_hi < kBwdStages) return IO_OK;
    IO_TRY(io_maxpool_bwd_t(Gd, reinterpret_cast<const uint32_t*>(c.ws + p.idx0), c.N, H0, H0, 64, Ge, c.st, c.dt()));
    {
        IoConvGeom g = io_geom_fwd(c.N, c.S, c.S, 8, 64, 7, 7, 2, 3);
        g.cr = net->stem.cin;
        if (stem_exact(c, net->stem) && io_stem_rows_ok(g) && c.N % c.G == 0) {
            const BnL& b = net->bn1;
            Tables t = c.tables(b);
            IO_TRY(io_bn_bwd_coefs_t(Ge, c.act(p.y0), c.N * H0 * H0, b.C, c.G, c.params + b.g_off, t.mean, t.rstd,
                                     c.grads + b.g_off, c.grads + b.b_off, c.buf(c.plan.coef), c.buf(c.plan.bn_partial),
                                     c.plan.bn_partial_floats, c.st, c.dt(), t.scale, t.shift));
            const size_t gs = (size_t)c.G * b.C;
            IoStemXb xb{};
            xb.y = (const float*)c.act(p.y0);
            xb.a = c.buf(c.plan.coef);
            xb.b = c.buf(c.plan.coef) + gs;
            xb.c = c.buf(c.plan.coef) + 2 * gs;
            xb.mean = t.mean;
            xb.scale = t.scale;
            xb.shift = t.shift;
            xb.G = c.G;
            IO_TRY(io_launch_stem_wgrad_rows(g, (const float*)x8, (const float*)Ge, c.buf(c.plan.stem_dwp),
                                             c.buf(c.plan.wg_partial), c.plan.wg_partial_bytes, c.st, &xb));
            return io_stem_unpack_grad(c.buf(c.plan.stem_dwp), c.grads + net->stem.w_off, net->stem.cout, 49,
                                       net->stem.cin, c.st);
        }
    }
    if (c.net->dtype == IO_BF16) {
        IoConvGeom g = io_geom_fwd(c.N, c.S, c.S, 8, 64, 7, 7, 2, 3);
        if (io_stem_wgrad_halo_ok(g, c.plan.wg_partial_bytes, c.G)) {
            const BnL& b = net->bn1;
            Tables t = c.tables(b);
            IO_TRY(io_bn_bwd_coefs_t(Ge, c.act(p.y0), c.N * H0 * H0, b.C, c.G, c.params + b.g_off, t.mean, t.rstd,
                                     c.grads + b.g_off, c.grads + b.b_off, c.buf(c.plan.coef), c.buf(c.plan.bn_partial),
                                     c.plan.bn_partial_floats, c.st, c.dt(), t.scale, t.shift));
            const size_t gs = (size_t)c.G * b.C;
            IoStemXb xb{};
            xb.y = (const float*)c.act(p.y0);
            xb.a = c.buf(c.plan.coef);
            xb.b = c.buf(c.plan.coef) + gs;
            xb.c = c.buf(c.plan.coef) + 2 * gs;
            xb.mean = t.mean;
            xb.scale = t.scale;
            xb.shift = t.shift;
            xb.G = c.G;
            return io_launch_stem_wgrad_halo(g, x8, Ge, c.grads + net->stem.w_off, c.buf(c.plan.wg_partial),
                                             c.plan.wg_partial_bytes, c.st, &xb);
        }
    }
    IO_TRY(bn_back(c, net->bn1, Ge, 1, nullptr, c.act(p.y0), c.N * H0 * H0, Ga, nullptr));
    IO_TRY(conv_wgrad(c, net->stem, x8, Ga, c.S));
    return IO_OK;
}

}

extern "C" io_net* io_net_create(int in_channels, int n_heads, const int* head_dims) {
    if (in_channels < 1 || in_channels > 5 || n_heads < 1 || n_heads > 2) {
        io_set_error("io_net_create: in_channels=%d (1..5), n_heads=%d (1..2)", in_channels, n_heads);
        return nullptr;
    }
    for (int i = 0; i < n_heads; ++i)
        if (head_dims[i] < 1 || head_dims[i] > 4 || (n_heads == 2 && i == 0 && head_dims[i] != 2)) {
            io_set_error("io_net_create: unsupported head dims");
            return nullptr;
        }
    io_net* net = new io_net();
    net->in_ch = in_channels;
    net->n_heads = n_heads;
    net->head_dims[0] = head_dims[0];
    net->head_dims[1] = n_heads > 1 ? head_dims[1] : 0;
    net->param_floats = 0;
    net->running_floats = 0;
    net->n_bn = 0;
    net->bn_channels = 0;
    net->stem = add_conv(net, "conv1", 64, in_channels, 7, 2, 3);
    net->stem.cin_store = 8;
    net->bn1 = add_bn(net, "bn1", 64);
    const int layers[4] = {3, 4, 6, 3}, planes[4] = {64, 128, 256, 512};
    int inC = 64;
    for (int li = 0; li < 4; ++li)
        for (int bi = 0; bi < layers[li]; ++bi) {
            Block b;
            char nm[64];
            b.planes = planes[li];
            b.inC = inC;
            b.stride = (bi == 0 && li > 0) ? 2 : 1;
            b.down = bi == 0;
            snprintf(nm, sizeof(nm), "layer%d.%d.conv1", li + 1, bi);
            b.c1 = add_conv(net, nm, b.planes, inC, 1, 1, 0);
            snprintf(nm, sizeof(nm), "layer%d.%d.bn1", li + 1, bi);
            b.b1 = add_bn(net, nm, b.planes);
            snprintf(nm, sizeof(nm), "layer%d.%d.conv2", li + 1, bi);
            b.c2 = add_conv(net, nm, b.planes, b.planes, 3, b.stride, 1);
            snprintf(nm, sizeof(nm), "layer%d.%d.bn2", li + 1, bi);
            b.b2 = add_bn(net, nm, b.planes);
            snprintf(nm, sizeof(nm), "layer%d.%d.conv3", li + 1, bi);
            b.c3 = add_conv(net, nm, b.planes * 4, b.planes, 1, 1, 0);
            snprintf(nm, sizeof(nm), "layer%d.%d.bn3", li + 1, bi);
            b.b3 = add_bn(net, nm, b.planes * 4);
            if (b.down) {
                snprintf(nm, sizeof(nm), "layer%d.%d.downsample.0", li + 1, bi);
                b.cd = add_conv(net, nm, b.planes * 4, inC, 1, b.stride, 0);
                snprintf(nm, sizeof(nm), "layer%d.%d.downsample.1", li + 1, bi);
                b.bd = add_bn(net, nm, b.planes * 4);
            }
            inC = b.planes * 4;
            net->blocks.push_back(b);
        }
    const char* hn1[1] = {"fc"};
    const char* hn2[2] = {"fc_occ", "fc_depth"};
    for (int i = 0; i < n_heads; ++i) {
        char nm[64];
        const char* base = n_heads == 1 ? hn1[0] : hn2[i];
        const long ws[2] = {head_dims[i], 2048};
        snprintf(nm, sizeof(nm), "%s.weight", base);
        add_tensor(net, nm, 3, 2, ws, (long)head_dims[i] * 2048, 2048, &net->fcw_off[i]);
        const long bs[1] = {head_dims[i]};
        snprintf(nm, sizeof(nm), "%s.bias", base);
        add_tensor(net, nm, 4, 1, bs, head_dims[i], head_dims[i], &net->fcb_off[i]);
    }
    return net;
}

extern "C" void io_net_destroy(io_net* net) { delete net; }
extern "C" int io_net_set_dtype(io_net* net, int dtype) {
    IO_REQUIRE(dtype == IO_F32 || dtype == IO_BF16, IO_ERR_SHAPE, "io_net_set_dtype: unknown dtype %d", dtype);
    net->dtype = dtype;
    return IO_OK;
}
extern "C" int io_net_get_dtype(const io_net* net) { return net->dtype; }
extern "C" long io_net_param_floats(const io_net* net) { return net->param_floats; }
extern "C" long io_net_running_floats(const io_net* net) { return net->running_floats; }
extern "C" int io_net_num_tensors(const io_net* net) { return (int)net->tensors.size(); }
extern "C" int io_net_num_logits(const io_net* net) { return net->head_dims[0] + net->head_dims[1]; }

extern "C" int io_net_tensor_info(const io_net* net, int i, io_tensor_info* out) {
    IO_REQUIRE(i >= 0 && i < (int)net->tensors.size(), IO_ERR_SHAPE, "tensor index %d out of range", i);
    *out = net->tensors[i];
    return IO_OK;
}

static int check_shape(int N, int S, int G) {
    IO_REQUIRE(S >= 32 && S % 32 == 0, IO_ERR_SHAPE, "input size S=%d must be a multiple of 32", S);
    IO_REQUIRE(N >= 1 && G >= 1 && G <= kMaxGroups && N % G == 0, IO_ERR_SHAPE, "N=%d G=%d (G<=%d, G | N)", N, G,
               kMaxGroups);
    IO_REQUIRE((double)N * S * S < 2.0e9, IO_ERR_SHAPE, "N=%d x S=%d: more than 2^31 input pixels", N, S);
    return IO_OK;
}

extern "C" size_t io_net_workspace_bytes(const io_net* net, int N, int S, int training) {
    if (check_shape(N, S, 1)) return 0;
    return make_plan(net, N, S, training != 0).total;
}

extern "C" long io_net_activation_offset(const io_net* net, int N, int S, int which) {
    if (check_shape(N, S, 1)) return -1;
    const Plan p = make_plan(net, N, S, true);
    const int nb = (int)net->blocks.size();
    if (which == 0) return (long)p.y0;
    if (which == 1) {
        io_set_error("io_net_activation_offset: relu(bn1(.)) is not stored (it is evaluated inside the pooling kernel)");
        return -1;
    }
    if (which == 2) return (long)p.p0;
    if (which >= 3 && which < 3 + nb) return (long)p.blk[which - 3].out;
    io_set_error("io_net_activation_offset: which=%d (0..%d)", which, 2 + nb);
    return -1;
}

static void fill_ctx(Ctx& c, io_net* net, const float* params, float* running, float* grads, int N, int S, int G,
                     bool training, void* ws, hipStream_t st, int SW = 0) {
    c.net = net;
    c.params = params;
    c.running = running;
    c.grads = grads;
    c.ws = (char*)ws;
    c.N = N; c.S = S; c.G = G;
    c.SW = SW > 0 ? SW : S;
    c.training = training;
    c.st = st;
    c.plan = make_plan(net, N, S, training, c.SW);
    c.chan_prefix.assign(net->n_bn, 0);
    std::vector<int> Cs(net->n_bn, 0);
    Cs[net->bn1.index] = net->bn1.C;
    for (const Block& b : net->blocks) {
        Cs[b.b1.index] = b.b1.C;
        Cs[b.b2.index] = b.b2.C;
        Cs[b.b3.index] = b.b3.C;
        if (b.down) Cs[b.bd.index] = b.bd.C;
    }
    long acc = 0;
    for (int i = 0; i < net->n_bn; ++i) { c.chan_prefix[i] = acc; acc += Cs[i]; }
}

extern "C" int io_net_forward(io_net* net, const float* params, float* running, const void* x8, int N, int S,
                              int G, int training, void* ws, size_t ws_bytes, float* logits, hipStream_t st) {
    IO_TRY(check_shape(N, S, G));
    IO_REQUIRE(training || G == 1, IO_ERR_SHAPE, "eval forward uses running statistics: G must be 1");
    Ctx c;
    fill_ctx(c, net, params, running, nullptr, N, S, G, training != 0, ws, st);
    IO_REQUIRE(ws_bytes >= c.plan.total, IO_ERR_WORKSPACE, "io_net_forward: workspace %zu < %zu bytes", ws_bytes,
               c.plan.total);
    return run_forward(c, x8, logits);
}

static int check_shape_hw(int N, int H, int W) {
    IO_REQUIRE(H >= 32 && H % 32 == 0 && W >= 32 && W % 32 == 0, IO_ERR_SHAPE,
               "input %d x %d: both sides must be multiples of 32 (five stride-2 stages)", H, W);
    IO_REQUIRE(N >= 1 && (double)N * H * W < 2.0e9, IO_ERR_SHAPE, "N=%d x %d x %d: more than 2^31 input pixels", N, H, W);
    return IO_OK;
}
extern "C" size_t io_net_workspace_bytes_hw(const io_net* net, int N, int H, int W) {
    if (check_shape_hw(N, H, W)) return 0;
// ... 38 lines not shown
```

instaorder_amd/csrc/stem.hip:

```cpp
#include <hip/hip_runtime.h>

#include <type_traits>

#include "io_common.h"

#ifndef IO_STEM_ABLATE
#define IO_STEM_ABLATE 0
#endif

typedef float f32x2 __attribute__((ext_vector_type(2)));
typedef float f32x4 __attribute__((ext_vector_type(4)));
typedef float f32x16 __attribute__((ext_vector_type(16)));

namespace {
constexpr int kCR = 5;
constexpr int kPW = 262;
constexpr int kPitch = kPW * kCR;
constexpr int kKB = 36;
constexpr int kBImg = 7 * 64 * kKB;
constexpr int kPix = 7 * kPW;
constexpr int kNT = 512;
constexpr int kRounds = (kPix + kNT - 1) / kNT;
constexpr int kPatch = kRounds * kNT * kCR;
constexpr int kRed = 2 * 4 * 64 * 2;
// ... 71 lines not shown
    const float bv = bias ? bias[ch] : 0.f;
    const float floor_v = relu ? 0.f : -__builtin_inff();
    f32x16 acc, pacc;
#pragma unroll
    for (int r = 0; r < 16; ++r) pacc[r] = 0.f;
    int cur = 0;
    auto mma_row = [&](int r) {
        const float* ar = sP + cur * kPatch + a_lane + r * kPitch;
        const float* br = b_lane + r * 64 * kKB;
#pragma unroll
        for (int q = 0; q < 4; ++q) {
            const f32x2 a0 = *reinterpret_cast<const f32x2*>(ar + 8 * q + 4 * h);
            const f32x2 a1 = *reinterpret_cast<const f32x2*>(ar + 8 * q + 4 * h + 2);
            const f32x4 b = *reinterpret_cast<const f32x4*>(br + 8 * q + 4 * h);
            acc = __builtin_amdgcn_mfma_f32_32x32x2f32(a0.x, b.x, acc, 0, 0, 0);
            acc = __builtin_amdgcn_mfma_f32_32x32x2f32(a0.y, b.y, acc, 0, 0, 0);
            acc = __builtin_amdgcn_mfma_f32_32x32x2f32(a1.x, b.z, acc, 0, 0, 0);
            acc = __builtin_amdgcn_mfma_f32_32x32x2f32(a1.y, b.w, acc, 0, 0, 0);
        }
        const f32x2 a = *reinterpret_cast<const f32x2*>(ar + 32 + 2 * h);
        const f32x2 b = *reinterpret_cast<const f32x2*>(br + 32 + 2 * h);
        acc = __builtin_amdgcn_mfma_f32_32x32x2f32(a.x, b.x, acc, 0, 0, 0);
        acc = __builtin_amdgcn_mfma_f32_32x32x2f32(a.y, b.y, acc, 0, 0, 0);
    };
    auto park = [&](int t) {
        float s = 0.f;
#pragma unroll
        for (int r = 0; r < 16; ++r) s += pacc[r];
        s += __shfl_xor(s, 32, 64);
        const float m = s * (1.f / 32.f);
        float q = 0.f;
#pragma unroll
        for (int r = 0; r < 16; ++r) q += (pacc[r] - m) * (pacc[r] - m);
        q += __shfl_xor(q, 32, 64);
        *reinterpret_cast<f32x2*>(sR + (((t & 1) * 4 + rg) * 64 + ch) * 2) = f32x2{m, q};
    };
    auto merge = [&](int t) {
        const float* rr = sR + ((t & 1) * 4 * 64 + ch) * 2;
        const f32x2 p0 = *reinterpret_cast<const f32x2*>(rr), p1 = *reinterpret_cast<const f32x2*>(rr + 128);
        const f32x2 p2 = *reinterpret_cast<const f32x2*>(rr + 256), p3 = *reinterpret_cast<const f32x2*>(rr + 384);
        const float mean = ((p0.x + p1.x) + (p2.x + p3.x)) * 0.25f;
        const float d0 = p0.x - mean, d1 = p1.x - mean, d2 = p2.x - mean, d3 = p3.x - mean;
        st_mean[(size_t)t * 64 + ch] = mean;
        st_m2[(size_t)t * 64 + ch] = ((p0.y + p1.y) + (p2.y + p3.y)) + 32.f * ((d0 * d0 + d1 * d1) + (d2 * d2 + d3 * d3));
    };
    auto store_half = [&](int t, int half) {
        float* o = out + ((size_t)t * 128 + rg * 32 + 4 * h) * 64 + ch;
#pragma unroll
        for (int r = 8 * half; r < 8 * half + 8; ++r) {
            const float v = pacc[r] + bv;
            o[(size_t)((r & 3) + 8 * (r >> 2)) * 64] = v < floor_v ? floor_v : v;
        }
    };
    auto body = [&](auto steady, int t) {
        constexpr bool STEADY = decltype(steady)::value;
        const bool have = STEADY || t < t_hi, prev = STEADY || (t > t_lo && t <= t_hi), prev2 = STEADY || t > t_lo + 1;
        const bool more = STEADY || t + 1 < t_hi;
        if (more && !(IO_STEM_ABLATE & 2)) fetch();
        __builtin_amdgcn_sched_barrier(0);
#pragma unroll
        for (int r = 0; r < 16; ++r) acc[r] = 0.f;
        if (have) mma_row(0);
        if (STATS && prev && !(IO_STEM_ABLATE & 4)) park(t - 1);
        if (have) mma_row(1);
        if (STATS && prev2 && !(IO_STEM_ABLATE & 4)) merge(t - 2);
        if (have) mma_row(2);
        if (prev && (!(IO_STEM_ABLATE & 1) || pacc[0] == 123.456f)) store_half(t - 1, 0);
        if (have) mma_row(3);
        if (prev && (!(IO_STEM_ABLATE & 1) || pacc[0] == 123.456f)) store_half(t - 1, 1);
        if (have) mma_row(4);
        if (more && !(IO_STEM_ABLATE & 2)) stage(cur ^ 1);
        if (have) mma_row(5);
        if (have) mma_row(6);
        __syncthreads();
        pacc = acc;
        cur ^= 1;
    };
    for (int t = t_lo; t <= t_hi + 1; ++t) {
        if (t > t_lo + 1 && t + 1 < t_hi) body(std::true_type{}, t);
        else body(std::false_type{}, t);
    }
}

constexpr int kWPitch = 1315;
constexpr int kWPatch = kRounds * kNT * kCR + 40;
constexpr int kWDy = 128 * 64;
constexpr size_t kWLds = (size_t)2 * (kWPatch + kWDy) * sizeof(float);

template <bool XB>
__global__ __launch_bounds__(kNT, 1) void stem_wgrad_rows_kernel(const float* __restrict__ x8, const float* __restrict__ dy,
                                                                 float* __restrict__ partial, int Hi, int Wi, int Ho, int Wo,
                                                                 int ntiles, int per_block, IoStemXb xb) {
    extern __shared__ __attribute__((aligned(16))) float smem[];
    float* sP = smem;
    float* sD = smem + 2 * kWPatch;
    const int tid = threadIdx.x, lane = tid & 63, wave = tid >> 6;
    const int l32 = lane & 31, h = lane >> 5;
    const int t_lo = blockIdx.x * per_block, t_hi = min(ntiles, t_lo + per_block);
    const int cbn = Wo >> 7;

    float pr[kRounds][kCR];
    f32x4 dr[4], yr[4], tb[6];
    int p_r[kRounds], p_c[kRounds], p_off[kRounds], p_dst[kRounds];
    bool p_ok[kRounds];
#pragma unroll
    for (int i = 0; i < kRounds; ++i) {
        const int p = tid + i * kNT;
        p_r[i] = p / kPW;
        p_c[i] = p - p_r[i] * kPW;
        p_off[i] = (p_r[i] * Wi + p_c[i]) * 8;
        p_dst[i] = p_r[i] * kWPitch + p_c[i] * kCR;
        if (p >= kPix || p_c[i] >= kPW - 1) p_r[i] = 1 << 20;
    }
    int f_cb = t_lo % cbn, f_ho = (t_lo / cbn) % Ho, f_n = (t_lo / cbn) / Ho;
    const float* f_dy = dy + (size_t)t_lo * kWDy + tid * 4;
    const float* f_y = XB ? xb.y + (size_t)t_lo * kWDy + tid * 4 : nullptr;
    int f_t = t_lo;
    auto fetch = [&]() {
        const int hi0 = 2 * f_ho - 3, wi0 = 256 * f_cb - 3;
        const float* base = x8 + (((ptrdiff_t)f_n * Hi + hi0) * Wi + wi0) * 8;
        if (++f_cb == cbn) {
            f_cb = 0;
            if (++f_ho == Ho) {
                f_ho = 0;
                ++f_n;
            }
        }
#pragma unroll
        for (int i = 0; i < kRounds; ++i) {
            const bool ok = (unsigned)(hi0 + p_r[i]) < (unsigned)Hi && (unsigned)(wi0 + p_c[i]) < (unsigned)Wi;
            const float* src = ok ? base + p_off[i] : x8;
            const f32x4 v = *reinterpret_cast<const f32x4*>(src);
            pr[i][0] = v.x; pr[i][1] = v.y; pr[i][2] = v.z; pr[i][3] = v.w;
            pr[i][4] = src[4];
            p_ok[i] = ok;
        }
#pragma unroll
        for (int i = 0; i < 4; ++i) dr[i] = *reinterpret_cast<const f32x4*>(f_dy + i * kNT * 4);
        f_dy += kWDy;
        if constexpr (XB) {
#pragma unroll
            for (int i = 0; i < 4; ++i) yr[i] = *reinterpret_cast<const f32x4*>(f_y + i * kNT * 4);
            f_y += kWDy;
            const int go = (f_t / xb.tiles_per_group) * 64 + (tid & 15) * 4;
            ++f_t;
            tb[0] = *reinterpret_cast<const f32x4*>(xb.a + go);
            tb[1] = *reinterpret_cast<const f32x4*>(xb.b + go);
            tb[2] = *reinterpret_cast<const f32x4*>(xb.c + go);
            tb[3] = *reinterpret_cast<const f32x4*>(xb.mean + go);
            tb[4] = *reinterpret_cast<const f32x4*>(xb.scale + go);
            tb[5] = *reinterpret_cast<const f32x4*>(xb.shift + go);
        }
    };
    auto stage = [&](int buf) {
        float* dst = sP + buf * kWPatch;
#pragma unroll
        for (int i = 0; i < kRounds; ++i)
#pragma unroll
            for (int c = 0; c < kCR; ++c) dst[p_dst[i] + c] = p_ok[i] ? pr[i][c] : 0.f;
        float* dd = sD + buf * kWDy + tid * 4;
#pragma unroll
        for (int i = 0; i < 4; ++i) {
            f32x4 v = dr[i];
            if constexpr (XB) {
#pragma unroll
                for (int e = 0; e < 4; ++e) {
                    const float act = __builtin_fmaf(yr[i][e] - tb[3][e], tb[4][e], tb[5][e]);
                    const float dz = act > 0.f ? v[e] : 0.f;
                    v[e] = __builtin_fmaf(tb[0][e], dz, __builtin_fmaf(tb[1][e], yr[i][e], tb[2][e]));
                }
            }
            *reinterpret_cast<f32x4*>(dd + i * kNT * 4) = v;
        }
    };

    fetch();
    stage(0);
    __syncthreads();

    const int j = wave * 32 + l32;
    const int jr = min(j, 7 * 7 * kCR - 1) / (7 * kCR), jk = min(j, 7 * 7 * kCR - 1) - jr * 7 * kCR;
    const int b_lane = jr * kWPitch + jk + 2 * kCR * h;
    const int a_lane = h * 64 + l32;
    f32x16 acc0, acc1;
#pragma unroll
    for (int r = 0; r < 16; ++r) acc0[r] = acc1[r] = 0.f;
    int cur = 0;
    auto mma_tile = [&]() {
        const float* pb = sP + cur * kWPatch + b_lane;
        const float* pa = sD + cur * kWDy + a_lane;
        float fb[2][8], fa0[2][8], fa1[2][8];
        auto read_chunk = [&](int c, int s) {
#pragma unroll
            for (int i = 0; i < 8; ++i) {
                fb[s][i] = pb[(c * 8 + i) * 4 * kCR];
                fa0[s][i] = pa[(c * 8 + i) * 128];
                fa1[s][i] = pa[(c * 8 + i) * 128 + 32];
            }
        };
        read_chunk(0, 0);
#pragma unroll
        for (int c = 0; c < 8; ++c) {
            if (c + 1 < 8) read_chunk(c + 1, (c + 1) & 1);
#pragma unroll
            for (int i = 0; i < 8; ++i) {
                acc0 = __builtin_amdgcn_mfma_f32_32x32x2f32(fa0[c & 1][i], fb[c & 1][i], acc0, 0, 0, 0);
                acc1 = __builtin_amdgcn_mfma_f32_32x32x2f32(fa1[c & 1][i], fb[c & 1][i], acc1, 0, 0, 0);
            }
            __builtin_amdgcn_sched_barrier(0);
        }
    };
    for (int t = t_lo; t < t_hi; ++t) {
        if (t + 1 < t_hi) {
            fetch();
            __builtin_amdgcn_sched_barrier(0);
            mma_tile();
            stage(cur ^ 1);
        } else {
            mma_tile();
        }
        __syncthreads();
        cur ^= 1;
    }
    float* o = partial + ((size_t)blockIdx.x * 64 + 4 * h) * 256 + j;
    const bool real = j < 7 * 7 * kCR;
#pragma unroll
    for (int r = 0; r < 16; ++r) {
        const int row = (r & 3) + 8 * (r >> 2);
        o[(size_t)row * 256] = real ? acc0[r] : 0.f;
        o[(size_t)(row + 32) * 256] = real ? acc1[r] : 0.f;
    }
}
}

bool io_stem_rows_ok(const IoConvGeom& g) {
    return g.cr == kCR && g.Ci == 8 && g.Co == 64 && g.Th == 7 && g.Tw == 7 && g.S == 7 && g.wT == 49 && g.is == 2 &&
           g.os == 1 && g.dh0 == -3 && g.dw0 == -3 && g.dhs == 1 && g.dws == 1 && g.r0 == 0 && g.rs == 1 && g.s0 == 0 &&
           g.ss == 1 && g.Ho == g.outH && g.Wo == g.outW && g.Wo % 128 == 0 && 2 * g.Ho == g.Hi && 2 * g.Wo == g.Wi &&
           (double)g.N * g.Ho * g.Wo < 2.0e9;
}

int io_launch_stem_rows(const IoConvGeom& g, const float* x8, const float* wp, float* out, float* st_mean, float* st_m2,
                        const float* bias, int relu, hipStream_t st) {
    IO_REQUIRE(io_stem_rows_ok(g), IO_ERR_SHAPE, "stem_rows: not the 7x7 stride-2 stem on whole 128-pixel output rows");
    const int ntiles = g.N * g.Ho * (g.Wo / 128);
    static std::atomic<unsigned long long> seen{0};
    static int ncu_of[64];
    int dev = 0;
    if (io_first_on_device(seen, &dev)) {
        hipDeviceProp_t prop;
        int n = hipGetDeviceProperties(&prop, dev) == hipSuccess ? prop.multiProcessorCount : 0;
        ncu_of[dev & 63] = n > 0 ? n : 256;
        (void)hipFuncSetAttribute((const void*)stem_rows_kernel<true>, hipFuncAttributeMaxDynamicSharedMemorySize, (int)kLds);
        (void)hipFuncSetAttribute((const void*)stem_rows_kernel<false>, hipFuncAttributeMaxDynamicSharedMemorySize, (int)kLds);
    }
    const int ncu = ncu_of[dev & 63] > 0 ? ncu_of[dev & 63] : 256;
    const int blocks = ntiles < ncu ? ntiles : ncu;
    const int per_block = (ntiles + blocks - 1) / blocks;
    const dim3 grid((unsigned)((ntiles + per_block - 1) / per_block));
    if (st_mean)
        hipLaunchKernelGGL(stem_rows_kernel<true>, grid, dim3(kNT), kLds, st, x8, wp, io_stem_kp(g.wT, g.cr), out, st_mean,
                           st_m2, bias, relu, g.Hi, g.Wi, g.Ho, g.Wo, ntiles, per_block);
    else
        hipLaunchKernelGGL(stem_rows_kernel<false>, grid, dim3(kNT), kLds, st, x8, wp, io_stem_kp(g.wT, g.cr), out, st_mean,
                           st_m2, bias, relu, g.Hi, g.Wi, g.Ho, g.Wo, ntiles, per_block);
    return io_check_launch("stem_rows");
}

int io_stem_wgrad_rows_max_blocks() { return 256; }

int io_launch_stem_wgrad_rows(const IoConvGeom& g, const float* x8, const float* dy, float* dwp, float* partial,
                              size_t partial_bytes, hipStream_t st, const IoStemXb* xb) {
    IO_REQUIRE(io_stem_rows_ok(g), IO_ERR_SHAPE, "stem_wgrad_rows: not the 7x7 stride-2 stem on whole 128-pixel output rows");
    const int ntiles = g.N * g.Ho * (g.Wo / 128);
    static std::atomic<unsigned long long> seen{0};
    static int ncu_of[64];
    int dev = 0;
    if (io_first_on_device(seen, &dev)) {
        hipDeviceProp_t prop;
        int n = hipGetDeviceProperties(&prop, dev) == hipSuccess ? prop.multiProcessorCount : 0;
        ncu_of[dev & 63] = (n <= 0 || n > io_stem_wgrad_rows_max_blocks()) ? io_stem_wgrad_rows_max_blocks() : n;
        (void)hipFuncSetAttribute((const void*)stem_wgrad_rows_kernel<false>, hipFuncAttributeMaxDynamicSharedMemorySize, (int)kWLds);
        (void)hipFuncSetAttribute((const void*)stem_wgrad_rows_kernel<true>, hipFuncAttributeMaxDynamicSharedMemorySize, (int)kWLds);
    }
    const int ncu = ncu_of[dev & 63] > 0 ? ncu_of[dev & 63] : io_stem_wgrad_rows_max_blocks();
    const int blocks = ntiles < ncu ? ntiles : ncu;
    const int per_block = (ntiles + blocks - 1) / blocks;
    const int grid = (ntiles + per_block - 1) / per_block;
    IO_REQUIRE(partial && partial_bytes >= (size_t)grid * 64 * 256 * sizeof(float), IO_ERR_WORKSPACE,
               "stem_wgrad_rows: workspace %zu < %zu bytes", partial_bytes, (size_t)grid * 64 * 256 * sizeof(float));
    IoStemXb x{};
    if (xb) {
        x = *xb;
        IO_REQUIRE(x.y && x.a && x.b && x.c && x.mean && x.scale && x.shift && x.G >= 1 && g.N % x.G == 0, IO_ERR_SHAPE,
                   "stem_wgrad_rows: the fused BatchNorm backward needs y, six [G][64] tables and G | N");
        x.tiles_per_group = ntiles / x.G;
    }
    const double Md = (double)g.N * g.Ho * g.Wo;
    {
        IoProfScope prof(IO_PROF_WGRAD_STEM, 2.0 * Md * 64 * 49.0 * kCR,
                         4.0 * (Md * 64 * (xb ? 2.0 : 1.0) + (double)g.N * g.Hi * g.Wi * 8 + 64.0 * 49 * kCR), st);
        if (xb)
            hipLaunchKernelGGL(stem_wgrad_rows_kernel<true>, dim3((unsigned)grid), dim3(kNT), kWLds, st, x8, dy, partial, g.Hi,
                               g.Wi, g.Ho, g.Wo, ntiles, per_block, x);
        else
            hipLaunchKernelGGL(stem_wgrad_rows_kernel<false>, dim3((unsigned)grid), dim3(kNT), kWLds, st, x8, dy, partial, g.Hi,
                               g.Wi, g.Ho, g.Wo, ntiles, per_block, x);
        const int rc = io_check_launch("stem_wgrad_rows");
        if (rc) return rc;
        return io_splitk_reduce(partial, dwp, (size_t)64 * 256 / 4, grid, st);
    }
}
```

instaorder_amd/engine.py:

```python
import ctypes as C

import torch

from . import _lib


def _ptr(t):
    return C.c_void_p(t.data_ptr()) if t is not None else C.c_void_p(0)


def _stream():
    return C.c_void_p(torch.cuda.current_stream().cuda_stream)


def _dev_f32(t, name):
    if not (t.is_cuda and t.dtype == torch.float32 and t.is_contiguous()):
        raise ValueError("%s must be a contiguous float32 tensor on the GPU" % name)
    return t


class Net(object):

    DTYPES = {"fp32": 0, "f32": 0, "float32": 0, "bf16": 1, "bfloat16": 1}

    def __init__(self, in_channels=5, num_classes=2, dtype="fp32"):
        self.lib = _lib.lib()
        if dtype not in self.DTYPES:
            raise ValueError("dtype must be 'fp32' or 'bf16', got %r" % (dtype,))
        self.dtype = "bf16" if self.DTYPES[dtype] else "fp32"
        heads = list(num_classes) if isinstance(num_classes, (list, tuple)) else [int(num_classes)]
        self.head_dims = heads
        arr = (C.c_int * len(heads))(*heads)
        self.handle = self.lib.io_net_create(int(in_channels), len(heads), arr)
        if not self.handle:
            raise RuntimeError("io_net_create failed: " + _lib.last_error())
        _lib.check(self.lib.io_net_set_dtype(self.handle, self.DTYPES[dtype]), "io_net_set_dtype")
        self.in_channels = int(in_channels)
        self.param_floats = int(self.lib.io_net_param_floats(self.handle))
        self.running_floats = int(self.lib.io_net_running_floats(self.handle))
        self.num_logits = int(self.lib.io_net_num_logits(self.handle))
        self.tensors = []
        info = _lib.TensorInfo()
        for i in range(self.lib.io_net_num_tensors(self.handle)):
            _lib.check(self.lib.io_net_tensor_info(self.handle, i, C.byref(info)), "io_net_tensor_info")
            self.tensors.append(dict(name=info.name.decode(), kind=info.kind,
                                     shape=tuple(info.shape[k] for k in range(info.ndim)),
                                     offset=int(info.offset), numel_storage=int(info.numel_storage),
                                     cin_storage=int(info.cin_storage), bn_index=int(info.bn_index),
                                     running_offset=int(info.running_offset)))

    def __del__(self):
        try:
            if getattr(self, "handle", None):
                self.lib.io_net_destroy(self.handle)
                self.handle = None
        except Exception:
            pass

    def workspace_bytes(self, N, S, training):
        n = int(self.lib.io_net_workspace_bytes(self.handle, int(N), int(S), int(bool(training))))
        if n == 0:
            raise RuntimeError("io_net_workspace_bytes: " + _lib.last_error())
        return n

    def activation_offset(self, N, S, which):
        off = int(self.lib.io_net_activation_offset(self.handle, int(N), int(S), int(which)))
        if off < 0:
            raise RuntimeError("io_net_activation_offset: " + _lib.last_error())
        return off

    def forward(self, params, running, x8, N, S, G, training, ws, logits):
        _lib.require_gpu()
        _lib.check(self.lib.io_net_forward(self.handle, _ptr(params), _ptr(running), _ptr(x8), int(N), int(S),
                                           int(G), int(bool(training)), _ptr(ws), ws.numel() * ws.element_size(),
                                           _ptr(logits), _stream()), "io_net_forward")

    def workspace_bytes_hw(self, N, H, W):
        n = int(self.lib.io_net_workspace_bytes_hw(self.handle, int(N), int(H), int(W)))
        if n == 0:
            raise RuntimeError("io_net_workspace_bytes_hw: " + _lib.last_error())
        return n

    def forward_eval_hw(self, params, running, x8, N, H, W, ws, logits):
        _lib.require_gpu()
        _lib.check(self.lib.io_net_forward_eval_hw(self.handle, _ptr(params), _ptr(running), _ptr(x8), int(N), int(H),
                                                   int(W), _ptr(ws), ws.numel() * ws.element_size(), _ptr(logits),
                                                   _stream()), "io_net_forward_eval_hw")

    def backward(self, params, grads, x8, dlogits, N, S, G, ws, stages=None):
        _lib.require_gpu()
        if stages is None:
            _lib.check(self.lib.io_net_backward(self.handle, _ptr(params), _ptr(grads), _ptr(x8), _ptr(dlogits),
                                                int(N), int(S), int(G), _ptr(ws), ws.numel() * ws.element_size(),
                                                _stream()), "io_net_backward")
        else:
            _lib.check(self.lib.io_net_backward_stages(self.handle, _ptr(params), _ptr(grads), _ptr(x8), _ptr(dlogits),
                                                       int(N), int(S), int(G), _ptr(ws), ws.numel() * ws.element_size(),
                                                       int(stages[0]), int(stages[1]), _stream()),
                       "io_net_backward_stages")

    @property
    def backward_stages(self):
        return int(self.lib.io_net_backward_num_stages(self.handle))


TORCH_DTYPE = {"fp32": torch.float32, "bf16": torch.bfloat16}


def pack_planes(planes, strides, N, H, W, out):
    _lib.require_gpu()
    n = len(planes)
    pa = (C.c_void_p * n)(*[t.data_ptr() + 4 * off for t, off in planes])
    sa = (C.c_long * n)(*[int(s) for s in strides])
    if out.dtype not in (torch.float32, torch.bfloat16) or not out.is_contiguous():
        raise ValueError("pack_planes: out must be a contiguous fp32 or bf16 tensor")
    _lib.check(_lib.lib().io_pack_planes_nhwc8_dt(pa, sa, n, int(N), int(H), int(W), _ptr(out),
                                                  1 if out.dtype == torch.bfloat16 else 0, _stream()),
               "io_pack_planes_nhwc8_dt")


def pack_nchw(x, out=None, dtype="fp32"):
    _dev_f32(x, "x")
    N, Cc, H, W = x.shape
    if out is None:
        out = torch.empty((N, H, W, 8), device=x.device, dtype=TORCH_DTYPE[dtype])
    pack_planes([(x, c * H * W) for c in range(Cc)], [Cc * H * W] * Cc, N, H, W, out)
    return out


def pack_pair_directions(rgb, modal1, modal2, out=None, dtype="fp32"):
    for t, nme in ((rgb, "rgb"), (modal1, "modal1"), (modal2, "modal2")):
        if t is not None:
            _dev_f32(t, nme)
    B, _, H, W = modal1.shape
    if out is None:
        out = torch.empty((2 * B, H, W, 8), device=modal1.device, dtype=TORCH_DTYPE[dtype])
    HW = H * W
    rgbp = [(rgb, c * HW) for c in range(3)] if rgb is not None else []
    st = [HW, HW] + [3 * HW] * len(rgbp)
    pack_planes([(modal1, 0), (modal2, 0)] + rgbp, st, B, H, W, out[:B])
    pack_planes([(modal2, 0), (modal1, 0)] + rgbp, st, B, H, W, out[B:])
# ... 137 lines not shown
```

instaorder_amd/supervised_order.py:

```python
import os

import torch
import torch.distributed as dist

from . import distributed_utils, engine
from .single_stage_model import SingleStageModel


def _dev(t, dtype=None):
    t = t.cuda(non_blocking=True)
    return t.to(dtype) if dtype is not None and t.dtype != dtype else t



def _force_overlap_requested():
    if os.environ.get("IO_COMM_OVERLAP", "1") != "force":
        return False
    if not (dist.is_available() and dist.is_initialized()):
        raise RuntimeError("IO_COMM_OVERLAP=force runs the staged gradient exchange (dist.all_reduce per backward stage): "
                           "initialise a process group first (torch.distributed.init_process_group, world_size >= 1) or "
                           "unset IO_COMM_OVERLAP")
    return True


class _OrderBase(SingleStageModel):

    KOCC = 0
    KDEP = 0

    def __init__(self, params, load_pretrain=None, dist_model=False):
        super(_OrderBase, self).__init__(params, dist_model)
        self.params = params
        self.use_rgb = params.get("use_rgb", False)
        want = 5 if self.use_rgb else 2
        if self.net.in_channels != want:
            raise ValueError("use_rgb=%s needs backbone_param.in_channels=%d, got %d"
                             % (self.use_rgb, want, self.net.in_channels))
        self._x8 = None
        self._use_graph = os.environ.get("IO_NO_GRAPH", "0") != "1"
        self._graph = None
        self._graph_ws = None
        self._dp_keep = None
        self._graph_key = None
        self._seen_key = None
        self._static = {}
        self._overlap_comm = os.environ.get("IO_COMM_OVERLAP", "1") != "0"
        self._force_overlap = _force_overlap_requested()
        self._buckets = None
        self._dp_graphs = None
        self._dp_key = None
        if load_pretrain is not None:
            self.load_pretrain(load_pretrain)

    def _static_copy(self, name, t):
        cur = self._static.get(name)
        if cur is None or cur.shape != t.shape or cur.dtype != t.dtype or cur.device != t.device:
            cur = torch.empty_like(t)
            self._static[name] = cur
            self._graph = None
            self._dp_graphs = None
        cur.copy_(t)
        return cur

    def _set_images(self, rgb, modal1, modal2):
        self.rgb = _dev(rgb, torch.float32).contiguous()
        self.modal1 = _dev(modal1, torch.float32).contiguous()
        self.modal2 = _dev(modal2, torch.float32).contiguous()
        B = self.rgb.shape[0]
        if self._x8 is None or self._x8.shape[0] != 2 * B or self._x8.shape[1:3] != self.rgb.shape[2:]:
            self._x8 = None
            self._graph = None
            self._dp_graphs = None
        self._x8 = engine.pack_pair_directions(self.rgb if self.use_rgb else None, self.modal1, self.modal2,
                                               self._x8, dtype=self.net.dtype)
        self.B = B

    def _loss_args(self, training):
        raise NotImplementedError

    def _loss(self, logits, training, want_grad):
        kw = self._loss_args(training)
        return engine.order_loss(logits, self.B, self.KOCC, self.KDEP, inv_world=1.0 / self.world_size,
                                 want_grad=want_grad, **kw)

    def _logs(self, losses):
        return None

    def _pack_return(self, losses):
        logs = self._logs(losses)
        out = {"loss": losses[0]}
        return (logs, out) if logs is not None else out

    def forward_only(self, ret_loss=True):
        with torch.no_grad():
            if self.net.training:
                logits = self.net.forward_packed(self._x8, groups=2)
            else:
                logits = self.net.forward_packed(self._x8, groups=1)
            self.last_logits = logits
            if not ret_loss:
                return {}
            losses, _ = self._loss(logits, False, False)
        logs = self._logs(losses)
        return (logs if logs is not None else {}), {"loss": losses[0]}

    def _fwd_loss_bwd(self, N, S):
        net = self.net
        logits, ws = net._run_forward(self._x8, N, S, 2, True)
        losses, dlogits = self._loss(logits, True, True)
        net._run_backward(self._x8, dlogits, N, S, 2, ws)
        return logits, losses, ws

    def _step_overlapped(self, N, S):
        net = self.net
        if self._buckets is None:
            self._buckets = distributed_utils.GradientBuckets(net)
        bk = self._buckets
        ns = bk.num_stages
        key = (N, S, self._x8.data_ptr(), net.flat_params.data_ptr())
        graphs_ok = self._use_graph and not engine.prof_active()
        if graphs_ok and self._dp_graphs is not None and self._dp_key == key:
            for s, g in enumerate(self._dp_graphs):
                g.replay()
                bk.launch(s)
            bk.finish()
            logits, losses = (t.clone() for t in self._dp_out)
            return logits, losses
        if graphs_ok and self._seen_key == key:
            graphs = None
            try:
                torch.cuda.synchronize()
                g0 = torch.cuda.CUDAGraph()
                with torch.cuda.graph(g0, capture_error_mode="thread_local"):
                    logits, ws = net._run_forward(self._x8, N, S, 2, True)
                    losses, dlogits = self._loss(logits, True, True)
                    net._run_backward(self._x8, dlogits, N, S, 2, ws, stages=(0, 1))
                graphs = [g0]
                for s in range(1, ns):
                    g = torch.cuda.CUDAGraph()
                    with torch.cuda.graph(g, pool=g0.pool(), capture_error_mode="thread_local"):
                        net._run_backward(self._x8, dlogits, N, S, 2, ws, stages=(s, s + 1))
                    graphs.append(g)
            except Exception as ex:
                graphs = None
                self._use_graph = False
                self._dp_graphs = None
                print("instaorder_amd: per-stage hipGraph capture disabled (%s)" % ex)
            if graphs is not None:
                self._dp_graphs, self._dp_key, self._dp_out, self._dp_keep = graphs, key, (logits, losses), (ws, dlogits)
                for s, g in enumerate(graphs):
                    g.replay()
                    bk.launch(s)
                bk.finish()
                return logits.clone(), losses.clone()
        lent = self._dp_keep[0] if (self._dp_graphs is not None and not net._pool.free) else None
        if lent is not None:
            net._pool.give(lent)
        logits, ws = net._run_forward(self._x8, N, S, 2, True)
        losses, dlogits = self._loss(logits, True, True)
        for s in range(ns):
            net._run_backward(self._x8, dlogits, N, S, 2, ws, stages=(s, s + 1))
            bk.launch(s)
        bk.finish()
        if ws is not lent:
            net._pool.give(ws)
        self._seen_key = key
        return logits, losses

    def step(self):
        net = self.net
        if not net.training:
            raise RuntimeError("step() needs switch_to('train')")
        N = 2 * self.B
        S = self._x8.shape[1]
        key = (N, S, self._x8.data_ptr(), net.flat_params.data_ptr())
        if (self.world_size > 1 or self._force_overlap) and self._overlap_comm:
            logits, losses = self._step_overlapped(N, S)
            self.last_logits = logits
            net.attach_grads()
            self.optim.step()
            return self._pack_return(losses)
        if self._use_graph and self._graph is not None and self._graph_key == key and not engine.prof_active():
            self._graph.replay()
            logits, losses = (t.clone() for t in self._graph_out)
        elif self._use_graph and self._seen_key == key and not engine.prof_active():
            try:
                ws_keep = None
                torch.cuda.synchronize()
                g = torch.cuda.CUDAGraph()
                with torch.cuda.graph(g, capture_error_mode="thread_local"):
                    logits, losses, ws_keep = self._fwd_loss_bwd(N, S)
                self._graph, self._graph_key, self._graph_out, self._graph_ws = g, key, (logits, losses), ws_keep
                g.replay()
                logits, losses = logits.clone(), losses.clone()
            except Exception as ex:
                self._use_graph = False
                self._graph = None
                print("instaorder_amd: hipGraph capture disabled (%s)" % ex)
                logits, losses, ws = self._fwd_loss_bwd(N, S)
                net._pool.give(ws)
        else:
            lent = self._graph_ws if (self._graph is not None and not net._pool.free) else None
            if lent is not None:
                net._pool.give(lent)
            logits, losses, ws = self._fwd_loss_bwd(N, S)
            if ws is not lent:
                net._pool.give(ws)
            self._seen_key = key
        self.last_logits = logits
        if self.world_size > 1:
            distributed_utils.average_gradients(self.model)
        net.attach_grads()
        self.optim.step()
        return self._pack_return(losses)


def _check_labels(t, lo, hi, what, is_overlap=None):
    if t is not None and torch.is_tensor(t) and not t.is_cuda and t.numel():
        if is_overlap is not None and torch.is_tensor(is_overlap):
            if is_overlap.is_cuda:
                is_overlap = is_overlap.cpu()
            live = (is_overlap.reshape(-1) == 0) | (is_overlap.reshape(-1) == 1)
            t = t.reshape(-1)[live]
            if not t.numel():
                return
        mn, mx = int(t.min()), int(t.max())
        if mn < lo or mx > hi:
            raise ValueError("%s: values must lie in [%d, %d], got [%d, %d]" % (what, lo, hi, mn, mx))


def _mirror_occ(occ_order):
    return occ_order[:, [1, 0]]


def _mirror_classes(order):
    return torch.where(order >= 2, order, 1 - order)


class InstaOrderNet_o(_OrderBase):
    KOCC = 2

    def set_input(self, rgb=None, modal1=None, modal2=None, occ_order=None):
        self._set_images(rgb, modal1, modal2)
        self.occ_order1 = _dev(occ_order, torch.float32)
        self.occ_order2 = _mirror_occ(self.occ_order1)
        self._occ_t = self._static_copy("occ", torch.cat([self.occ_order1, self.occ_order2], 0))

    def _loss_args(self, training):
        return dict(occ_target=self._occ_t)


class InstaOrderNet_od(_OrderBase):
# ... 429 lines not shown
```

Baseline: 1826 pairs/s.

## Exploit paired-instance input structure in stem conv forward and weight-gradient

Adds a pair-aware stem path that treats the two instances of each pair together. The first two input channels of the 7x7 filter are re-expressed as sum and difference weights, so the shared channels are computed once per pair. New forward (with BN statistics) and wgrad kernels process pair tiles, with pack and unpack kernels to convert the filter and gradient layouts. It is enabled by default in training through an environment flag and relies on assumptions about how the paired inputs relate, which adds some risk for other input forms.

```diff
diff --git a/include/instaorder_hip.h b/include/instaorder_hip.h
--- a/include/instaorder_hip.h
+++ b/include/instaorder_hip.h
@@ -146,6 +146,8 @@
 #define IO_DTYPE_BF16 1
 int io_net_set_dtype(io_net* net, int dtype);
 int io_net_get_dtype(const io_net* net);
+int io_net_set_pair_input(io_net* net, int on);
+int io_net_get_pair_input(const io_net* net);
 int io_pack_planes_nhwc8_dt(const float* const* planes, const long* sample_strides, int nplanes, int N, int H, int W,
                             void* out, int dtype, hipStream_t stream);
 int io_conv2d_fwd_dt(const void* x, const void* w, void* y, int N, int H, int W, int Cin, int Cout, int R, int S,
@@ -239,11 +241,24 @@
                               float* workspace, size_t workspace_floats, float* packed, hipStream_t stream);
 int io_stem_wgrad_exact(const float* x8, const float* dy, float* dw, int N, int H, int W, int real_channels,
                         void* workspace, size_t workspace_bytes, float* packed, hipStream_t stream);
+int io_stem_pair_form(int N, int H, int W, int real_channels, int G);
+int io_stem_pairs_fwd_bnstats_exact(const float* x8, const float* w, float* y, int N, int H, int W, int real_channels, int G,
+                                    const float* gamma, const float* beta, float* running_mean, float* running_var,
+                                    float momentum, float eps, float* mean, float* rstd, float* scale, float* shift,
+                                    float* workspace, size_t workspace_floats, float* packed, hipStream_t stream);
 int io_stem_wgrad_exact_bn(const float* x8, const float* da, const float* y, float* dw, int N, int H, int W,
                            int real_channels, int G, const float* gamma, const float* mean, const float* rstd,
                            const float* scale, const float* shift, float* dgamma, float* dbeta, float* coef,
                            float* bn_partial, size_t bn_partial_floats, void* workspace, size_t workspace_bytes,
                            float* packed, hipStream_t stream);
+
+int io_stem_pairs_wgrad_exact(const float* x8, const float* dy, float* dw, int N, int H, int W, int real_channels,
+                              void* workspace, size_t workspace_bytes, float* packed, hipStream_t stream);
+int io_stem_pairs_wgrad_exact_bn(const float* x8, const float* da, const float* y, float* dw, int N, int H, int W,
+                                 int real_channels, int G, const float* gamma, const float* mean, const float* rstd,
+                                 const float* scale, const float* shift, float* dgamma, float* dbeta, float* coef,
+                                 float* bn_partial, size_t bn_partial_floats, void* workspace, size_t workspace_bytes,
+                                 float* packed, hipStream_t stream);
 
 size_t io_bn_tile_partial_floats(int M, int C, int G);
 int io_bn_bwd_coefs_dt(const void* dz, const void* y, int M, int C, int G, const float* gamma, const float* mean,
diff --git a/instaorder_amd/_lib.py b/instaorder_amd/_lib.py
--- a/instaorder_amd/_lib.py
+++ b/instaorder_amd/_lib.py
@@ -117,6 +117,8 @@
     "io_net_backward_stages": (_I, [_P, _P, _P, _P, _P, _I, _I, _I, _P, _Z, _I, _I, _P]),
     "io_net_set_dtype": (_I, [_P, _I]),
     "io_net_get_dtype": (_I, [_P]),
+    "io_net_set_pair_input": (_I, [_P, _I]),
+    "io_net_get_pair_input": (_I, [_P]),
     "io_pack_planes_nhwc8_dt": (_I, [_P, _P, _I, _I, _I, _I, _P, _I, _P]),
     "io_conv2d_fwd_dt": (_I, [_P, _P, _P, _I, _I, _I, _I, _I, _I, _I, _I, _I, _I, _I, _P]),
     "io_conv2d_dgrad_dt": (_I, [_P, _P, _P, _P, _P, _I, _I, _I, _I, _I, _I, _I, _I, _I, _I, _P]),
@@ -148,7 +150,13 @@
     "io_stem_wgrad_exact_workspace_bytes": (_Z, [_I, _I, _I, _I]),
     "io_stem_fwd_bnstats_exact": (_I, [_P, _P, _P, _I, _I, _I, _I, _I, _P, _P, _P, _P, _F, _F, _P, _P, _P, _P, _P, _Z, _P,
                                        _P]),
+    "io_stem_pair_form": (_I, [_I, _I, _I, _I, _I]),
+    "io_stem_pairs_fwd_bnstats_exact": (_I, [_P, _P, _P, _I, _I, _I, _I, _I, _P, _P, _P, _P, _F, _F, _P, _P, _P, _P, _P, _Z,
+                                             _P, _P]),
     "io_stem_wgrad_exact": (_I, [_P, _P, _P, _I, _I, _I, _I, _P, _Z, _P, _P]),
+    "io_stem_pairs_wgrad_exact": (_I, [_P, _P, _P, _I, _I, _I, _I, _P, _Z, _P, _P]),
+    "io_stem_pairs_wgrad_exact_bn": (_I, [_P, _P, _P, _P, _I, _I, _I, _I, _I, _P, _P, _P, _P, _P, _P, _P, _P, _P, _Z, _P, _Z,
+                                          _P, _P]),
     "io_stem_wgrad_exact_bn": (_I, [_P, _P, _P, _P, _I, _I, _I, _I, _I, _P, _P, _P, _P, _P, _P, _P, _P, _P, _Z, _P, _Z, _P,
                                     _P]),
     "io_stem_wgrad_bn_bf16": (_I, [_P, _P, _P, _P, _I, _I, _I, _I, _P, _P, _P, _P, _P, _P, _P, _P, _P, _Z, _P, _Z, _P]),
diff --git a/instaorder_amd/csrc/capi.hip b/instaorder_amd/csrc/capi.hip
--- a/instaorder_amd/csrc/capi.hip
+++ b/instaorder_amd/csrc/capi.hip
@@ -470,6 +470,31 @@
     return io_bn_finalize_tiles(tmean, tm2, M, 64, G, gamma, beta, running_mean, running_var, momentum, eps, mean, rstd,
                                 scale, shift, st);
 }
+extern "C" int io_stem_pair_form(int N, int H, int W, int real_channels, int G) {
+    if (N < 1 || H < 1 || W < 1 || real_channels < 1 || real_channels > 8) return 0;
+    return io_stem_pairs_ok(stem_geom_exact(N, H, W, real_channels), G) ? 1 : 0;
+}
+extern "C" int io_stem_pairs_fwd_bnstats_exact(const float* x8, const float* w, float* y, int N, int H, int W,
+                                               int real_channels, int G, const float* gamma, const float* beta,
+                                               float* running_mean, float* running_var, float momentum, float eps,
+                                               float* mean, float* rstd, float* scale, float* shift, float* workspace,
+                                               size_t workspace_floats, float* packed, hipStream_t st) {
+    IO_REQUIRE(io_stem_pair_form(N, H, W, real_channels, G), IO_ERR_SHAPE,
+               "stem_pairs: needs 5 real channels, 256 | H, W, an even N and G of 1 or 2 (else: io_stem_fwd_bnstats_exact)");
+    IoConvGeom g = stem_geom_exact(N, H, W, real_channels);
+    const int M = N * g.Ho * g.Wo;
+    const size_t need = io_conv2d_bnstats_workspace_floats(N, H, W, 64, 7, 7, 2, 3, G);
+    IO_REQUIRE(workspace_floats >= need && packed, IO_ERR_WORKSPACE, "stem_pairs: workspace %zu < %zu floats",
+               workspace_floats, need);
+    int rc = io_stem_pack_filter_pairs(w, packed, st);
+    if (rc) return rc;
+    float* tmean = workspace;
+    float* tm2 = workspace + need / 2;
+    rc = io_launch_stem_pairs_rows(g, x8, packed, y, tmean, tm2, st);
+    if (rc) return rc;
+    return io_bn_finalize_tiles(tmean, tm2, M, 64, G, gamma, beta, running_mean, running_var, momentum, eps, mean, rstd,
+                                scale, shift, st);
+}
 extern "C" int io_stem_wgrad_exact(const float* x8, const float* dy, float* dw, int N, int H, int W, int real_channels,
                                    void* ws, size_t ws_bytes, float* packed, hipStream_t st) {
     IO_REQUIRE(real_channels >= 1 && real_channels <= 8 && packed, IO_ERR_SHAPE, "stem_wgrad_exact: real_channels=%d (1..8)",
@@ -506,6 +531,41 @@
     rc = io_launch_stem_wgrad_rows(g, x8, da, packed, (float*)ws, ws_bytes, st, &xb);
     if (rc) return rc;
     return io_stem_unpack_grad(packed, dw, 64, 49, real_channels, st);
+}
+
+extern "C" int io_stem_pairs_wgrad_exact(const float* x8, const float* dy, float* dw, int N, int H, int W, int real_channels,
+                                         void* ws, size_t ws_bytes, float* packed, hipStream_t st) {
+    IO_REQUIRE(io_stem_pair_form(N, H, W, real_channels, 1) && packed, IO_ERR_SHAPE,
+               "stem_pairs_wgrad: needs 5 real channels, 256 | H, W and an even N (else: io_stem_wgrad_exact)");
+    IoConvGeom g = stem_geom_exact(N, H, W, real_channels);
+    int rc = io_launch_stem_wgrad_pairs(g, x8, dy, packed, (float*)ws, ws_bytes, st, nullptr);
+    if (rc) return rc;
+    return io_stem_unpack_grad_pairs(packed, dw, st);
+}
+extern "C" int io_stem_pairs_wgrad_exact_bn(const float* x8, const float* da, const float* y, float* dw, int N, int H, int W,
+                                            int real_channels, int G, const float* gamma, const float* mean,
+                                            const float* rstd, const float* scale, const float* shift, float* dgamma,
+                                            float* dbeta, float* coef, float* bn_partial, size_t bn_partial_floats, void* ws,
+                                            size_t ws_bytes, float* packed, hipStream_t st) {
+    IO_REQUIRE(io_stem_pair_form(N, H, W, real_channels, G) && packed && coef, IO_ERR_SHAPE,
+               "stem_pairs_wgrad_bn: needs 5 real channels, 256 | H, W, an even N and G of 1 or 2 (else: io_stem_wgrad_exact_bn)");
+    IoConvGeom g = stem_geom_exact(N, H, W, real_channels);
+    const int M = N * g.Ho * g.Wo;
+    int rc = io_bn_bwd_coefs_t(da, y, M, 64, G, gamma, mean, rstd, dgamma, dbeta, coef, bn_partial, bn_partial_floats, st, IO_F32,
+                               scale, shift);
+    if (rc) return rc;
+    IoStemXb xb{};
+    xb.y = y;
+    xb.a = coef;
+    xb.b = coef + (size_t)G * 64;
+    xb.c = coef + (size_t)2 * G * 64;
+    xb.mean = mean;
+    xb.scale = scale;
+    xb.shift = shift;
+    xb.G = G;
+    rc = io_launch_stem_wgrad_pairs(g, x8, da, packed, (float*)ws, ws_bytes, st, &xb);
+    if (rc) return rc;
+    return io_stem_unpack_grad_pairs(packed, dw, st);
 }
 
 extern "C" size_t io_stem_wgrad_bf16_workspace_bytes(void) { return io_stem_wgrad_halo_partial_bytes(); }
diff --git a/instaorder_amd/csrc/io_common.h b/instaorder_amd/csrc/io_common.h
--- a/instaorder_amd/csrc/io_common.h
+++ b/instaorder_amd/csrc/io_common.h
@@ -195,6 +195,11 @@
 bool io_stem_rows_ok(const IoConvGeom& g);
 int io_launch_stem_rows(const IoConvGeom& g, const float* x8, const float* wp, float* out, float* st_mean, float* st_m2,
                         const float* bias, int relu, hipStream_t st);
+bool io_stem_pairs_ok(const IoConvGeom& g, int G);
+int io_stem_pack_filter_pairs(const float* w, float* wimg, hipStream_t st);
+int io_launch_stem_pairs_rows(const IoConvGeom& g, const float* x8, const float* wimg, float* out, float* st_mean,
+                              float* st_m2, hipStream_t st);
+int io_stem_unpack_grad_pairs(const float* dwp, float* dw, hipStream_t st);
 int io_stem_wgrad_rows_max_blocks();
 struct IoStemXb {
     const float *y, *a, *b, *c, *mean, *scale, *shift;
@@ -202,6 +207,8 @@
 };
 int io_launch_stem_wgrad_rows(const IoConvGeom& g, const float* x8, const float* dy, float* dwp, float* partial,
                               size_t partial_bytes, hipStream_t st, const IoStemXb* xb = nullptr);
+int io_launch_stem_wgrad_pairs(const IoConvGeom& g, const float* x8, const float* dy, float* dwp, float* partial,
+                               size_t partial_bytes, hipStream_t st, const IoStemXb* xb = nullptr);
 size_t io_stem_wgrad_halo_partial_bytes();
 bool io_stem_wgrad_halo_ok(const IoConvGeom& g, size_t partial_bytes, int G);
 int io_launch_stem_wgrad_halo(const IoConvGeom& g, const void* x8, const void* dz, float* dw, float* partial, size_t partial_bytes,
diff --git a/instaorder_amd/csrc/misc.hip b/instaorder_amd/csrc/misc.hip
--- a/instaorder_amd/csrc/misc.hip
+++ b/instaorder_amd/csrc/misc.hip
@@ -977,6 +977,43 @@
     const int o = ot / T, tp = ot - o * T;
     dw[idx] = ch < cr ? dwp[(size_t)o * kp + tp * cr + ch] : 0.f;
 }
+__global__ __launch_bounds__(256) void stem_pack_filter_pairs_kernel(const float* __restrict__ w, float* __restrict__ wimg) {
+    const int idx = blockIdx.x * 256 + threadIdx.x;
+    if (idx >= 7 * 64 * 36) return;
+    const int k = idx % 36, rc = idx / 36, o = rc & 63, r = rc >> 6;
+    const int s = k < 28 ? k >> 2 : k - 28, c = k < 28 ? k & 3 : 4;
+    float v = 0.f;
+    if (s < 7) {
+        const float* t = w + ((size_t)o * 49 + r * 7 + s) * 8;
+        v = c == 0 ? 0.5f * (t[0] + t[1]) : c == 4 ? 0.5f * (t[0] - t[1]) : t[c + 1];
+    }
+    wimg[idx] = v;
+}
+__global__ __launch_bounds__(256) void stem_unpack_grad_pairs_kernel(const float* __restrict__ dwp, float* __restrict__ dw) {
+    const int idx = blockIdx.x * 256 + threadIdx.x;
+    if (idx >= 64 * 49 * 8) return;
+    const int ch = idx & 7, ot = idx >> 3;
+    const int o = ot / 49, tp = ot - o * 49;
+    const float* row = dwp + (size_t)o * 256;
+    float v = 0.f;
+    if (ch < 2) {
+        const float ps = row[tp * 4], qd = row[196 + tp];
+        v = 0.5f * (ch == 0 ? ps + qd : ps - qd);
+    } else if (ch < 5) {
+        v = row[tp * 4 + ch - 1];
+    }
+    dw[idx] = v;
+}
+}
+
+int io_stem_unpack_grad_pairs(const float* dwp, float* dw, hipStream_t st) {
+    hipLaunchKernelGGL(stem_unpack_grad_pairs_kernel, dim3(io_cdiv((long)64 * 49 * 8, 256)), dim3(256), 0, st, dwp, dw);
+    return io_check_launch("stem_unpack_grad_pairs");
+}
+
+int io_stem_pack_filter_pairs(const float* w, float* wimg, hipStream_t st) {
+    hipLaunchKernelGGL(stem_pack_filter_pairs_kernel, dim3(io_cdiv((long)7 * 64 * 36, 256)), dim3(256), 0, st, w, wimg);
+    return io_check_launch("stem_pack_filter_pairs");
 }
 
 int io_stem_pack_filter(const float* w, float* wp, int O, int T, int cr, hipStream_t st) {
diff --git a/instaorder_amd/csrc/net.hip b/instaorder_amd/csrc/net.hip
--- a/instaorder_amd/csrc/net.hip
+++ b/instaorder_amd/csrc/net.hip
@@ -32,6 +32,7 @@
 
 struct io_net {
     int dtype = IO_F32;
+    int pair_input = 0;
     int in_ch, n_heads, head_dims[2];
     ConvL stem;
     BnL bn1;
@@ -296,6 +297,11 @@
     const void* w = c.wop(L.w_off);
     if (stem_exact(c, L)) {
         g.cr = L.cin;
+        if (c.net->pair_input && c.training && stats && L.cin == 5 && !xf && !xr && io_stem_pairs_ok(g, c.G)) {
+            IO_TRY(io_stem_pack_filter_pairs(c.params + L.w_off, c.buf(c.plan.stem_wp), c.st));
+            return io_launch_stem_pairs_rows(g, (const float*)x, c.buf(c.plan.stem_wp), (float*)y, c.buf(c.plan.tile_mean),
+                                             c.buf(c.plan.tile_m2), c.st);
+        }
         IO_TRY(io_stem_pack_filter(c.params + L.w_off, c.buf(c.plan.stem_wp), L.cout, L.k * L.k, L.cin, c.st));
         w = c.buf(c.plan.stem_wp);
     }
@@ -788,6 +794,11 @@
             xb.scale = t.scale;
             xb.shift = t.shift;
             xb.G = c.G;
+            if (c.net->pair_input && net->stem.cin == 5 && io_stem_pairs_ok(g, c.G)) {
+                IO_TRY(io_launch_stem_wgrad_pairs(g, (const float*)x8, (const float*)Ge, c.buf(c.plan.stem_dwp),
+                                                  c.buf(c.plan.wg_partial), c.plan.wg_partial_bytes, c.st, &xb));
+                return io_stem_unpack_grad_pairs(c.buf(c.plan.stem_dwp), c.grads + net->stem.w_off, c.st);
+            }
             IO_TRY(io_launch_stem_wgrad_rows(g, (const float*)x8, (const float*)Ge, c.buf(c.plan.stem_dwp),
                                              c.buf(c.plan.wg_partial), c.plan.wg_partial_bytes, c.st, &xb));
             return io_stem_unpack_grad(c.buf(c.plan.stem_dwp), c.grads + net->stem.w_off, net->stem.cout, 49,
@@ -898,6 +909,11 @@
     return IO_OK;
 }
 extern "C" int io_net_get_dtype(const io_net* net) { return net->dtype; }
+extern "C" int io_net_set_pair_input(io_net* net, int on) {
+    net->pair_input = on ? 1 : 0;
+    return IO_OK;
+}
+extern "C" int io_net_get_pair_input(const io_net* net) { return net->pair_input; }
 extern "C" long io_net_param_floats(const io_net* net) { return net->param_floats; }
 extern "C" long io_net_running_floats(const io_net* net) { return net->running_floats; }
 extern "C" int io_net_num_tensors(const io_net* net) { return (int)net->tensors.size(); }
diff --git a/instaorder_amd/csrc/stem.hip b/instaorder_amd/csrc/stem.hip
--- a/instaorder_amd/csrc/stem.hip
+++ b/instaorder_amd/csrc/stem.hip
@@ -177,6 +177,177 @@
     }
 }
 
+constexpr int kPairU = 2 * kCR;
+constexpr int kRedP = 2 * kRed;
+constexpr size_t kLdsP = (size_t)(kBImg + 2 * kPatch + kRedP) * sizeof(float);
+
+__global__ __launch_bounds__(kNT, 1) void stem_pairs_rows_kernel(const float* __restrict__ x8, const float* __restrict__ wimg,
+                                                                 float* __restrict__ out, float* __restrict__ st_mean,
+                                                                 float* __restrict__ st_m2, int Hi, int Wi, int Ho, int Wo,
+                                                                 int ntiles, int per_block) {
+    extern __shared__ __attribute__((aligned(16))) float smem[];
+    float* sB = smem;
+    float* sP = smem + kBImg;
+    float* sR = sP + 2 * kPatch;
+    const int tid = threadIdx.x, lane = tid & 63, wave = tid >> 6;
+    const int rg = wave & 3, cg = wave >> 2;
+    const int l32 = lane & 31, h = lane >> 5;
+    const int t_lo = blockIdx.x * per_block, t_hi = min(ntiles, t_lo + per_block);
+    if (t_lo >= t_hi) return;
+    const int cbn = Wo >> 7;
+
+    for (int idx = tid; idx < kBImg / 4; idx += kNT)
+        reinterpret_cast<f32x4*>(sB)[idx] = reinterpret_cast<const f32x4*>(wimg)[idx];
+
+    float pr[kRounds][kCR];
+    int p_r[kRounds], p_c[kRounds], p_off[kRounds];
+    bool p_ok[kRounds];
+#pragma unroll
+    for (int i = 0; i < kRounds; ++i) {
+        const int p = tid + i * kNT;
+        p_r[i] = p / kPW;
+        p_c[i] = p - p_r[i] * kPW;
+        p_off[i] = (p_r[i] * Wi + p_c[i]) * 8;
+        if (p >= kPix || p_c[i] >= kPW - 1) p_r[i] = 1 << 20;
+    }
+    int f_cb = t_lo % cbn, f_ho = (t_lo / cbn) % Ho, f_n = (t_lo / cbn) / Ho;
+    auto fetch = [&]() {
+        const int hi0 = 2 * f_ho - 3, wi0 = 256 * f_cb - 3;
+        const float* base = x8 + (((ptrdiff_t)f_n * Hi + hi0) * Wi + wi0) * 8;
+        if (++f_cb == cbn) {
+            f_cb = 0;
+            if (++f_ho == Ho) {
+                f_ho = 0;
+                ++f_n;
+            }
+        }
+#pragma unroll
+        for (int i = 0; i < kRounds; ++i) {
+            const bool ok = (unsigned)(hi0 + p_r[i]) < (unsigned)Hi && (unsigned)(wi0 + p_c[i]) < (unsigned)Wi;
+            const float* src = ok ? base + p_off[i] : x8;
+            const f32x4 v = *reinterpret_cast<const f32x4*>(src);
+            pr[i][0] = v.x; pr[i][1] = v.y; pr[i][2] = v.z; pr[i][3] = v.w;
+            pr[i][4] = src[4];
+            p_ok[i] = ok;
+        }
+    };
+    auto stage = [&](int buf) {
+        float* dst = sP + buf * kPatch + (tid >> 1) * kPairU + (tid & 1) * 4;
+        float* dd = sP + buf * kPatch + (tid >> 1) * kPairU + 8 + (tid & 1);
+#pragma unroll
+        for (int i = 0; i < kRounds; ++i) {
+            const float m1 = p_ok[i] ? pr[i][0] : 0.f, m2 = p_ok[i] ? pr[i][1] : 0.f;
+            *reinterpret_cast<f32x2*>(dst + i * kNT * kCR) = f32x2{m1 + m2, p_ok[i] ? pr[i][2] : 0.f};
+            *reinterpret_cast<f32x2*>(dst + i * kNT * kCR + 2) = f32x2{p_ok[i] ? pr[i][3] : 0.f, p_ok[i] ? pr[i][4] : 0.f};
+            dd[i * kNT * kCR] = m1 - m2;
+        }
+    };
+
+    fetch();
+    stage(0);
+    __syncthreads();
+
+    const int a_lane = kPairU * (rg * 32 + l32);
+    const float* b_lane = sB + (cg * 32 + l32) * kKB;
+    const int ch = cg * 32 + l32;
+    f32x16 accp, accq, pacc0, pacc1;
+#pragma unroll
+    for (int r = 0; r < 16; ++r) pacc0[r] = pacc1[r] = 0.f;
+    int cur = 0;
+    auto mma_row = [&](int r) {
+        const float* ar = sP + cur * kPatch + a_lane + r * kPitch;
+        const float* br = b_lane + r * 64 * kKB;
+#pragma unroll
+        for (int q = 0; q < 3; ++q) {
+            const f32x2 a0 = *reinterpret_cast<const f32x2*>(ar + kPairU * q + 4 * h);
+            const f32x2 a1 = *reinterpret_cast<const f32x2*>(ar + kPairU * q + 4 * h + 2);
+            const f32x4 b = *reinterpret_cast<const f32x4*>(br + 8 * q + 4 * h);
+            accp = __builtin_amdgcn_mfma_f32_32x32x2f32(a0.x, b.x, accp, 0, 0, 0);
+            accp = __builtin_amdgcn_mfma_f32_32x32x2f32(a0.y, b.y, accp, 0, 0, 0);
+            accp = __builtin_amdgcn_mfma_f32_32x32x2f32(a1.x, b.z, accp, 0, 0, 0);
+            accp = __builtin_amdgcn_mfma_f32_32x32x2f32(a1.y, b.w, accp, 0, 0, 0);
+        }
+        const f32x2 a = *reinterpret_cast<const f32x2*>(ar + 3 * kPairU + 2 * h);
+        const f32x2 b = *reinterpret_cast<const f32x2*>(br + 24 + 2 * h);
+        accp = __builtin_amdgcn_mfma_f32_32x32x2f32(a.x, b.x, accp, 0, 0, 0);
+        accp = __builtin_amdgcn_mfma_f32_32x32x2f32(a.y, b.y, accp, 0, 0, 0);
+        const f32x2 d0 = *reinterpret_cast<const f32x2*>(ar + 2 * kPairU * h + 8);
+        const f32x2 d1 = *reinterpret_cast<const f32x2*>(ar + 2 * kPairU * h + kPairU + 8);
+        const f32x4 bq = *reinterpret_cast<const f32x4*>(br + 28 + 4 * h);
+        accq = __builtin_amdgcn_mfma_f32_32x32x2f32(d0.x, bq.x, accq, 0, 0, 0);
+        accq = __builtin_amdgcn_mfma_f32_32x32x2f32(d0.y, bq.y, accq, 0, 0, 0);
+        accq = __builtin_amdgcn_mfma_f32_32x32x2f32(d1.x, bq.z, accq, 0, 0, 0);
+        accq = __builtin_amdgcn_mfma_f32_32x32x2f32(d1.y, bq.w, accq, 0, 0, 0);
+    };
+    auto park = [&](int t, int s, const f32x16& pa) {
+        float sum = 0.f;
+#pragma unroll
+        for (int r = 0; r < 16; ++r) sum += pa[r];
+        sum += __shfl_xor(sum, 32, 64);
+        const float m = sum * (1.f / 32.f);
+        float q = 0.f;
+#pragma unroll
+        for (int r = 0; r < 16; ++r) q += (pa[r] - m) * (pa[r] - m);
+        q += __shfl_xor(q, 32, 64);
+        *reinterpret_cast<f32x2*>(sR + ((((t & 1) * 2 + s) * 4 + rg) * 64 + ch) * 2) = f32x2{m, q};
+    };
+    auto merge = [&](int t, int s) {
+        const float* rr = sR + (((t & 1) * 2 + s) * 4 * 64 + ch) * 2;
+        const f32x2 p0 = *reinterpret_cast<const f32x2*>(rr), p1 = *reinterpret_cast<const f32x2*>(rr + 128);
+        const f32x2 p2 = *reinterpret_cast<const f32x2*>(rr + 256), p3 = *reinterpret_cast<const f32x2*>(rr + 384);
+        const float mean = ((p0.x + p1.x) + (p2.x + p3.x)) * 0.25f;
+        const float d0 = p0.x - mean, d1 = p1.x - mean, d2 = p2.x - mean, d3 = p3.x - mean;
+        const size_t o = ((size_t)t + (size_t)s * ntiles) * 64 + ch;
+        st_mean[o] = mean;
+        st_m2[o] = ((p0.y + p1.y) + (p2.y + p3.y)) + 32.f * ((d0 * d0 + d1 * d1) + (d2 * d2 + d3 * d3));
+    };
+    auto store_half = [&](int t, int s, int half, const f32x16& pa) {
+        float* o = out + (((size_t)t + (size_t)s * ntiles) * 128 + rg * 32 + 4 * h) * 64 + ch;
+#pragma unroll
+        for (int r = 8 * half; r < 8 * half + 8; ++r) o[(size_t)((r & 3) + 8 * (r >> 2)) * 64] = pa[r];
+    };
+    auto body = [&](auto steady, int t) {
+        constexpr bool STEADY = decltype(steady)::value;
+        const bool have = STEADY || t < t_hi, prev = STEADY || (t > t_lo && t <= t_hi), prev2 = STEADY || t > t_lo + 1;
+        const bool more = STEADY || t + 1 < t_hi;
+        if (more) fetch();
+        __builtin_amdgcn_sched_barrier(0);
+#pragma unroll
+        for (int r = 0; r < 16; ++r) accp[r] = accq[r] = 0.f;
+        if (have) mma_row(0);
+        if (prev) {
+            park(t - 1, 0, pacc0);
+            park(t - 1, 1, pacc1);
+        }
+        if (have) mma_row(1);
+        if (prev2) {
+            merge(t - 2, 0);
+            merge(t - 2, 1);
+        }
+        if (prev) store_half(t - 1, 0, 0, pacc0);
+        if (have) mma_row(2);
+        if (prev) store_half(t - 1, 0, 1, pacc0);
+        if (have) mma_row(3);
+        if (prev) store_half(t - 1, 1, 0, pacc1);
+        if (have) mma_row(4);
+        if (prev) store_half(t - 1, 1, 1, pacc1);
+        if (have) mma_row(5);
+        if (more) stage(cur ^ 1);
+        if (have) mma_row(6);
+        __syncthreads();
+#pragma unroll
+        for (int r = 0; r < 16; ++r) {
+            pacc0[r] = accp[r] + accq[r];
+            pacc1[r] = accp[r] - accq[r];
+        }
+        cur ^= 1;
+    };
+    for (int t = t_lo; t <= t_hi + 1; ++t) {
+        if (t > t_lo + 1 && t + 1 < t_hi) body(std::true_type{}, t);
+        else body(std::false_type{}, t);
+    }
+}
+
 constexpr int kWPitch = 1315;
 constexpr int kWPatch = kRounds * kNT * kCR + 40;
 constexpr int kWDy = 128 * 64;
@@ -324,6 +495,201 @@
         const int row = (r & 3) + 8 * (r >> 2);
         o[(size_t)row * 256] = real ? acc0[r] : 0.f;
         o[(size_t)(row + 32) * 256] = real ? acc1[r] : 0.f;
+    }
+}
+
+constexpr int kWUV = 128 * 128;
+constexpr int kWTab = 2 * 6 * 64;
+constexpr int kWCh = 4;
+constexpr size_t kWLdsP = (size_t)(2 * kWPatch + kWUV + kWTab) * sizeof(float);
+static_assert(kWLdsP <= kWLds + kWTab * sizeof(float), "the pair form: the LDS of stem_wgrad_rows_kernel + 3 KB of tables");
+
+template <bool XB>
+__global__ __launch_bounds__(kNT, 1) void stem_wgrad_pairs_kernel(const float* __restrict__ x8, const float* __restrict__ dy,
+                                                                  float* __restrict__ partial, int Hi, int Wi, int Ho, int Wo,
+                                                                  int ntiles, int per_block, IoStemXb xb) {
+    extern __shared__ __attribute__((aligned(16))) float smem[];
+    float* sP = smem;
+    float* sD = smem + 2 * kWPatch;
+    float* sT = sD + kWUV;
+    const int tid = threadIdx.x, lane = tid & 63, wave = tid >> 6;
+    const int l32 = lane & 31, h = lane >> 5;
+    const int t_lo = blockIdx.x * per_block, t_hi = min(ntiles, t_lo + per_block);
+    const int cbn = Wo >> 7;
+
+    float pr[kRounds][kCR];
+    f32x4 dr[2][4], yr[2][4];
+    int p_r[kRounds], p_c[kRounds], p_off[kRounds], p_dst[kRounds];
+    bool p_ok[kRounds];
+#pragma unroll
+    for (int i = 0; i < kRounds; ++i) {
+        const int p = tid + i * kNT;
+        p_r[i] = p / kPW;
+        p_c[i] = p - p_r[i] * kPW;
+        p_off[i] = (p_r[i] * Wi + p_c[i]) * 8;
+        p_dst[i] = p_r[i] * kWPitch + p_c[i] * kCR;
+        if (p >= kPix || p_c[i] >= kPW - 1) p_r[i] = 1 << 20;
+    }
+    if constexpr (XB) {
+        const float* const src[6] = {xb.a, xb.b, xb.c, xb.mean, xb.scale, xb.shift};
+        for (int idx = tid; idx < kWTab; idx += kNT) {
+            const int s = idx / 384, k = (idx >> 6) % 6, c = idx & 63;
+            sT[idx] = src[k][s * (xb.G - 1) * 64 + c];
+        }
+    }
+    int f_cb = t_lo % cbn, f_ho = (t_lo / cbn) % Ho, f_n = (t_lo / cbn) / Ho;
+    const size_t second = (size_t)ntiles * kWDy;
+    const float* f_dy = dy + (size_t)t_lo * kWDy + tid * 4;
+    const float* f_y = XB ? xb.y + (size_t)t_lo * kWDy + tid * 4 : nullptr;
+    auto fetch = [&]() {
+        const int hi0 = 2 * f_ho - 3, wi0 = 256 * f_cb - 3;
+        const float* base = x8 + (((ptrdiff_t)f_n * Hi + hi0) * Wi + wi0) * 8;
+        if (++f_cb == cbn) {
+            f_cb = 0;
+            if (++f_ho == Ho) {
+                f_ho = 0;
+                ++f_n;
+            }
+        }
+#pragma unroll
+        for (int i = 0; i < kRounds; ++i) {
+            const bool ok = (unsigned)(hi0 + p_r[i]) < (unsigned)Hi && (unsigned)(wi0 + p_c[i]) < (unsigned)Wi;
+            const float* src = ok ? base + p_off[i] : x8;
+            const f32x4 v = *reinterpret_cast<const f32x4*>(src);
+            pr[i][0] = v.x; pr[i][1] = v.y; pr[i][2] = v.z; pr[i][3] = v.w;
+            pr[i][4] = src[4];
+            p_ok[i] = ok;
+        }
+#pragma unroll
+        for (int i = 0; i < 4; ++i) {
+            dr[0][i] = *reinterpret_cast<const f32x4*>(f_dy + i * kNT * 4);
+            dr[1][i] = *reinterpret_cast<const f32x4*>(f_dy + second + i * kNT * 4);
+        }
+        f_dy += kWDy;
+        if constexpr (XB) {
+#pragma unroll
+            for (int i = 0; i < 4; ++i) {
+                yr[0][i] = *reinterpret_cast<const f32x4*>(f_y + i * kNT * 4);
+                yr[1][i] = *reinterpret_cast<const f32x4*>(f_y + second + i * kNT * 4);
+            }
+            f_y += kWDy;
+        }
+    };
+    auto stage_patch = [&](int buf) {
+        float* dst = sP + buf * kWPatch;
+#pragma unroll
+        for (int i = 0; i < kRounds; ++i) {
+            const float m1 = p_ok[i] ? pr[i][0] : 0.f, m2 = p_ok[i] ? pr[i][1] : 0.f;
+            dst[p_dst[i]] = m1 + m2;
+#pragma unroll
+            for (int c = 1; c < 4; ++c) dst[p_dst[i] + c] = p_ok[i] ? pr[i][c + 1] : 0.f;
+            dst[p_dst[i] + 4] = m1 - m2;
+        }
+    };
+    auto stage_uv = [&]() {
+        float* dd = sD + (tid >> 4) * 128 + (tid & 15) * 4;
+        f32x4 tb[2][6];
+        if constexpr (XB) {
+#pragma unroll
+            for (int s = 0; s < 2; ++s)
+#pragma unroll
+                for (int k = 0; k < 6; ++k) tb[s][k] = *reinterpret_cast<const f32x4*>(sT + (s * 6 + k) * 64 + (tid & 15) * 4);
+        }
+#pragma unroll
+        for (int i = 0; i < 4; ++i) {
+            f32x4 v[2] = {dr[0][i], dr[1][i]};
+            if constexpr (XB) {
+#pragma unroll
+                for (int s = 0; s < 2; ++s)
+#pragma unroll
+                    for (int e = 0; e < 4; ++e) {
+                        const float act = __builtin_fmaf(yr[s][i][e] - tb[s][3][e], tb[s][4][e], tb[s][5][e]);
+                        const float dz = act > 0.f ? v[s][e] : 0.f;
+                        v[s][e] = __builtin_fmaf(tb[s][0][e], dz, __builtin_fmaf(tb[s][1][e], yr[s][i][e], tb[s][2][e]));
+                    }
+            }
+            *reinterpret_cast<f32x4*>(dd + i * 32 * 128) = v[0] + v[1];
+            *reinterpret_cast<f32x4*>(dd + i * 32 * 128 + 64) = v[0] - v[1];
+        }
+    };
+
+    if (t_lo < t_hi) {
+        fetch();
+        stage_patch(0);
+    }
+    __syncthreads();
+    if (t_lo < t_hi) stage_uv();
+    __syncthreads();
+
+    const bool qwave = wave >= 6, third = wave < 2;
+    auto p_col = [&](int j) {
+        const int jc = min(j, 195), r = jc / 28, k = jc - r * 28;
+        return r * kWPitch + (k >> 2) * kCR + (k & 3);
+    };
+    const int j = (qwave ? wave - 6 : wave) * 32 + l32;
+    const int jq = min(j, 48);
+    const int b_lane = (qwave ? (jq / 7) * kWPitch + (jq % 7) * kCR + 4 : p_col(j)) + 2 * kCR * h;
+    const int b_lane2 = p_col(192 + l32) + 2 * kCR * h;
+    const int a_lane = h * 128 + l32 + (qwave ? 64 : 0);
+    const int a_lane2 = h * 128 + l32 + 32 * wave;
+    f32x16 acc0, acc1, acc2;
+#pragma unroll
+    for (int r = 0; r < 16; ++r) acc0[r] = acc1[r] = acc2[r] = 0.f;
+    int cur = 0;
+    auto mma_tile = [&](auto with_third) {
+        constexpr bool T3 = decltype(with_third)::value;
+        const float* pb = sP + cur * kWPatch;
+        float fb[2][kWCh], fb2[2][kWCh], fa0[2][kWCh], fa1[2][kWCh], fa2[2][kWCh];
+        auto read_chunk = [&](int c, int s) {
+#pragma unroll
+            for (int i = 0; i < kWCh; ++i) {
+                fb[s][i] = pb[b_lane + (c * kWCh + i) * 4 * kCR];
+                fa0[s][i] = sD[a_lane + (c * kWCh + i) * 256];
+                fa1[s][i] = sD[a_lane + (c * kWCh + i) * 256 + 32];
+                if constexpr (T3) {
+                    fb2[s][i] = pb[b_lane2 + (c * kWCh + i) * 4 * kCR];
+                    fa2[s][i] = sD[a_lane2 + (c * kWCh + i) * 256];
+                }
+            }
+        };
+        read_chunk(0, 0);
+#pragma unroll
+        for (int c = 0; c < 64 / kWCh; ++c) {
+            if (c + 1 < 64 / kWCh) read_chunk(c + 1, (c + 1) & 1);
+#pragma unroll
+            for (int i = 0; i < kWCh; ++i) {
+                acc0 = __builtin_amdgcn_mfma_f32_32x32x2f32(fa0[c & 1][i], fb[c & 1][i], acc0, 0, 0, 0);
+                acc1 = __builtin_amdgcn_mfma_f32_32x32x2f32(fa1[c & 1][i], fb[c & 1][i], acc1, 0, 0, 0);
+                if constexpr (T3) acc2 = __builtin_amdgcn_mfma_f32_32x32x2f32(fa2[c & 1][i], fb2[c & 1][i], acc2, 0, 0, 0);
+            }
+            __builtin_amdgcn_sched_barrier(0);
+        }
+    };
+    for (int t = t_lo; t < t_hi; ++t) {
+        const bool more = t + 1 < t_hi;
+        if (more) {
+            fetch();
+            __builtin_amdgcn_sched_barrier(0);
+        }
+        if (third) mma_tile(std::true_type{});
+        else mma_tile(std::false_type{});
+        if (more) stage_patch(cur ^ 1);
+        __syncthreads();
+        if (more) stage_uv();
+        __syncthreads();
+        cur ^= 1;
+    }
+    float* o = partial + ((size_t)blockIdx.x * 64 + 4 * h) * 256;
+    const int col = qwave ? 196 + j : j;
+    const bool wr = qwave ? j < 60 : true, real = qwave ? j < 49 : true;
+#pragma unroll
+    for (int r = 0; r < 16; ++r) {
+        const int row = (r & 3) + 8 * (r >> 2);
+        if (wr) {
+            o[(size_t)row * 256 + col] = real ? acc0[r] : 0.f;
+            o[(size_t)(row + 32) * 256 + col] = real ? acc1[r] : 0.f;
+        }
+        if (third && l32 < 4) o[(size_t)(row + 32 * wave) * 256 + 192 + l32] = acc2[r];
     }
 }
 }
@@ -362,6 +728,37 @@
     return io_check_launch("stem_rows");
 }
 
+bool io_stem_pairs_ok(const IoConvGeom& g, int G) {
+    return io_stem_rows_ok(g) && g.N >= 2 && g.N % 2 == 0 && (G == 1 || G == 2);
+}
+
+int io_launch_stem_pairs_rows(const IoConvGeom& g, const float* x8, const float* wimg, float* out, float* st_mean,
+                              float* st_m2, hipStream_t st) {
+    IO_REQUIRE(io_stem_pairs_ok(g, 1) && st_mean && st_m2, IO_ERR_SHAPE,
+               "stem_pairs_rows: needs the 7x7 stride-2 stem on whole 128-pixel output rows, an even batch and statistics");
+    const int ntiles = (g.N / 2) * g.Ho * (g.Wo / 128);
+    static std::atomic<unsigned long long> seen{0};
+    static int ncu_of[64];
+    int dev = 0;
+    if (io_first_on_device(seen, &dev)) {
+        hipDeviceProp_t prop;
+        int n = hipGetDeviceProperties(&prop, dev) == hipSuccess ? prop.multiProcessorCount : 0;
+        ncu_of[dev & 63] = n > 0 ? n : 256;
+        (void)hipFuncSetAttribute((const void*)stem_pairs_rows_kernel, hipFuncAttributeMaxDynamicSharedMemorySize, (int)kLdsP);
+    }
+    const int ncu = ncu_of[dev & 63] > 0 ? ncu_of[dev & 63] : 256;
+    const int blocks = ntiles < ncu ? ntiles : ncu;
+    const int per_block = (ntiles + blocks - 1) / blocks;
+    const dim3 grid((unsigned)((ntiles + per_block - 1) / per_block));
+    const double Md = (double)g.N * g.Ho * g.Wo;
+    const double flops = 2.0 * Md * 64 * 49.0 * kCR;
+    IoProfScope prof(IO_PROF_CONV_STEM, flops, 4.0 * (Md * 64 + 0.5 * (double)g.N * g.Hi * g.Wi * 8 + 64.0 * 49 * kCR), st,
+                     0.5 * flops);
+    hipLaunchKernelGGL(stem_pairs_rows_kernel, grid, dim3(kNT), kLdsP, st, x8, wimg, out, st_mean, st_m2, g.Hi, g.Wi, g.Ho,
+                       g.Wo, ntiles, per_block);
+    return io_check_launch("stem_pairs_rows");
+}
+
 int io_stem_wgrad_rows_max_blocks() { return 256; }
 
 int io_launch_stem_wgrad_rows(const IoConvGeom& g, const float* x8, const float* dy, float* dwp, float* partial,
@@ -406,3 +803,45 @@
         return io_splitk_reduce(partial, dwp, (size_t)64 * 256 / 4, grid, st);
     }
 }
+
+int io_launch_stem_wgrad_pairs(const IoConvGeom& g, const float* x8, const float* dy, float* dwp, float* partial,
+                               size_t partial_bytes, hipStream_t st, const IoStemXb* xb) {
+    IO_REQUIRE(io_stem_pairs_ok(g, xb ? xb->G : 1), IO_ERR_SHAPE,
+               "stem_wgrad_pairs: needs the 7x7 stride-2 stem on whole 128-pixel output rows, an even batch and G of 1 or 2");
+    const int ntiles = (g.N / 2) * g.Ho * (g.Wo / 128);
+    static std::atomic<unsigned long long> seen{0};
+    static int ncu_of[64];
+    int dev = 0;
+    if (io_first_on_device(seen, &dev)) {
+        hipDeviceProp_t prop;
+        int n = hipGetDeviceProperties(&prop, dev) == hipSuccess ? prop.multiProcessorCount : 0;
+        ncu_of[dev & 63] = (n <= 0 || n > io_stem_wgrad_rows_max_blocks()) ? io_stem_wgrad_rows_max_blocks() : n;
+        (void)hipFuncSetAttribute((const void*)stem_wgrad_pairs_kernel<false>, hipFuncAttributeMaxDynamicSharedMemorySize, (int)kWLdsP);
+        (void)hipFuncSetAttribute((const void*)stem_wgrad_pairs_kernel<true>, hipFuncAttributeMaxDynamicSharedMemorySize, (int)kWLdsP);
+    }
+    const int ncu = ncu_of[dev & 63] > 0 ? ncu_of[dev & 63] : io_stem_wgrad_rows_max_blocks();
+    const int blocks = ntiles < ncu ? ntiles : ncu;
+    const int per_block = (ntiles + blocks - 1) / blocks;
+    const int grid = (ntiles + per_block - 1) / per_block;
+    IO_REQUIRE(partial && partial_bytes >= (size_t)grid * 64 * 256 * sizeof(float), IO_ERR_WORKSPACE,
+               "stem_wgrad_pairs: workspace %zu < %zu bytes", partial_bytes, (size_t)grid * 64 * 256 * sizeof(float));
+    IoStemXb x{};
+    if (xb) {
+        x = *xb;
+        IO_REQUIRE(x.y && x.a && x.b && x.c && x.mean && x.scale && x.shift, IO_ERR_SHAPE,
+                   "stem_wgrad_pairs: the fused BatchNorm backward needs y and six [G][64] tables");
+    }
+    const double Md = (double)g.N * g.Ho * g.Wo;
+    const double flops = 2.0 * Md * 64 * 49.0 * kCR;
+    IoProfScope prof(IO_PROF_WGRAD_STEM, flops,
+                     4.0 * (Md * 64 * (xb ? 2.0 : 1.0) + 0.5 * (double)g.N * g.Hi * g.Wi * 8 + 64.0 * 49 * kCR), st, 0.5 * flops);
+    if (xb)
+        hipLaunchKernelGGL(stem_wgrad_pairs_kernel<true>, dim3((unsigned)grid), dim3(kNT), kWLdsP, st, x8, dy, partial, g.Hi,
+                           g.Wi, g.Ho, g.Wo, ntiles, per_block, x);
+    else
+        hipLaunchKernelGGL(stem_wgrad_pairs_kernel<false>, dim3((unsigned)grid), dim3(kNT), kWLdsP, st, x8, dy, partial, g.Hi,
+                           g.Wi, g.Ho, g.Wo, ntiles, per_block, x);
+    const int rc = io_check_launch("stem_wgrad_pairs");
+    if (rc) return rc;
+    return io_splitk_reduce(partial, dwp, (size_t)64 * 256 / 4, grid, st);
+}
diff --git a/instaorder_amd/engine.py b/instaorder_amd/engine.py
--- a/instaorder_amd/engine.py
+++ b/instaorder_amd/engine.py
@@ -57,6 +57,13 @@
         except Exception:
             pass
 
+    def set_pair_input(self, on):
+        _lib.check(self.lib.io_net_set_pair_input(self.handle, int(bool(on))), "io_net_set_pair_input")
+
+    @property
+    def pair_input(self):
+        return bool(self.lib.io_net_get_pair_input(self.handle))
+
     def workspace_bytes(self, N, S, training):
         n = int(self.lib.io_net_workspace_bytes(self.handle, int(N), int(S), int(bool(training))))
         if n == 0:
diff --git a/instaorder_amd/supervised_order.py b/instaorder_amd/supervised_order.py
--- a/instaorder_amd/supervised_order.py
+++ b/instaorder_amd/supervised_order.py
@@ -1,3 +1,4 @@
+import contextlib
 import os
 
 import torch
@@ -37,6 +38,7 @@
             raise ValueError("use_rgb=%s needs backbone_param.in_channels=%d, got %d"
                              % (self.use_rgb, want, self.net.in_channels))
         self._x8 = None
+        self._pair_stem = os.environ.get("IO_PAIR_STEM", "1") != "0"
         self._use_graph = os.environ.get("IO_NO_GRAPH", "0") != "1"
         self._graph = None
         self._graph_ws = None
@@ -91,10 +93,20 @@
         out = {"loss": losses[0]}
         return (logs, out) if logs is not None else out
 
+    @contextlib.contextmanager
+    def _pair_batch(self):
+        plan = self.net.plan
+        plan.set_pair_input(self._pair_stem)
+        try:
+            yield
+        finally:
+            plan.set_pair_input(False)
+
     def forward_only(self, ret_loss=True):
         with torch.no_grad():
             if self.net.training:
-                logits = self.net.forward_packed(self._x8, groups=2)
+                with self._pair_batch():
+                    logits = self.net.forward_packed(self._x8, groups=2)
             else:
                 logits = self.net.forward_packed(self._x8, groups=1)
             self.last_logits = logits
@@ -168,6 +180,10 @@
         return logits, losses
 
     def step(self):
+        with self._pair_batch():
+            return self._step()
+
+    def _step(self):
         net = self.net
         if not net.training:
             raise RuntimeError("step() needs switch_to('train')")
```

After: 1844 pairs/s, median of 6. Within noise of the previous version (+1.0%).
